# open-flash/swf-renderer

Measured on AMD Instinct MI355X. Metric: Mpixels/sec rasterized @ 4K, 10k-edge synthetic shape set, higher is better.
Workload: dtype i32+f64(exact integers)/u8

## Files before the change

### swf_renderer_amd/csrc/device_types.hpp

```cpp
#pragma once

#include <stdint.h>

#include "../../include/swfr.h"

namespace swfr {

constexpr int TILE_W = 64;
constexpr int TILE_H = 16;
constexpr int STRIP_H = 8;
constexpr int STRIPS_PER_TILE = TILE_H / STRIP_H;

struct DevEdge {
    int32_t ytop, ybot;
    int32_t x1, y1;
    int32_t dir;
    int32_t pad;
    int64_t ex;
    int64_t dy;
    int64_t dq, dr;
    double inv_dy;
    double inv_dx;
    int64_t fr;
    int64_t r15;
    int32_t fq, q15;
};
static_assert(sizeof(DevEdge) == 96, "DevEdge layout");

struct FastEdge {
    int32_t x1, a0, DX, D;
    double invD;
    int32_t q15, r15;
    int32_t hq, hr;
    int32_t dqf, drf;
    int32_t ytop, ybot;
    int32_t dir, fq;
    double invW, fr;
};
static_assert(sizeof(FastEdge) == 80, "FastEdge layout");

using DevPath = swfr_path;

enum : uint32_t { ROW_EMPTY = 0, ROW_FULL = 1, ROW_SUB = 2 };
constexpr uint32_t REC_FULL = 0x80000000u;
constexpr uint32_t REC_CELLS = 0x40000000u;
constexpr int ROWS_CHUNK = 64;

enum : uint32_t { PATH_OP_MASK = 0x0fu, PATH_OP_LERP = 0x10u, PATH_OP_GROUP_BEGIN = 0x20u, PATH_OP_GROUP_END = 0x40u, PATH_OP_MASKED = 0x80u };
enum : uint32_t { BE_BOXES = 1u, BE_LERP = 2u, BE_SOLID = 4u, BE_OPAQUE_COVER = 8u  };

struct ChunkInfo {
    uint32_t path, first_row, rec_base, rows;
    uint32_t slot0;
    uint32_t first_edge, n_edges;
    uint32_t pad;
};

struct BandSlot {
    uint32_t path;
    uint32_t slot;
    uint32_t band;
    uint32_t pad;
};

struct DevBitmap {
    const uint32_t* pixels;
    uint32_t width, height;
};

struct DevFilter {
    int32_t on, cw, ch, xbits, ybits;
    uint32_t x_off, y_off;
    int32_t m00, m01, m10, m11;
    int32_t pad;
    int64_t base_x, base_y;
    const uint32_t* pixels;
    uint32_t width, height;
    uint32_t extend;
    uint32_t kind;
    uint32_t nearest;
    uint32_t pad2;
};
static_assert(sizeof(DevFilter) == 96, "DevFilter layout");

struct DevGradient {
    int64_t base_x, base_y;
    int32_t m00, m01, m10, m11;
    int32_t c1x, c1y, c1r, dx, dy, dr;
    int32_t n_intervals, extend;
    double a, inva, mindr;
    int32_t x[SWFR_MAX_STOPS + 2];
    float ramp[SWFR_MAX_STOPS + 1][8];
    uint16_t col[SWFR_MAX_STOPS + 2][4];
    int32_t x_min, pad;
};

struct Cell {
    uint32_t w;
};
static_assert(sizeof(Cell) == 4, "Cell layout");
constexpr int MAX_PATH_WIDTH = 8192;
constexpr int CELL_H = 16384;
constexpr Cell make_cell_v(int col_rel, int v) { return Cell{((uint32_t)col_rel << 19) | ((uint32_t)v & 0x7ffffu)}; }
constexpr Cell make_cell(int col_rel, int ch, int ua) { return make_cell_v(col_rel, ch * CELL_H + ua); }
constexpr int cell_col(Cell c) { return (int)(c.w >> 19); }
constexpr int cell_ua(Cell c) { return (int)(c.w << 18) >> 18; }
constexpr int cell_ch(Cell c) { return (((int)(c.w << 13) >> 13) - cell_ua(c)) >> 14; }
constexpr int MAX_CELLS_PER_EDGE_ROW = 17;

struct RowInfo2 {
    uint32_t off;
    uint16_t n;
    uint16_t mode;
};
enum : uint32_t { ROW_DEFER = 3,
                  ROW_FOREIGN = 4 };

struct BandEntry2 {
    int16_t x_min, x_max, y_min, y_max;
    uint32_t flags;
    uint32_t solid;
    uint32_t style;
    uint32_t first_edge, n_edges;
    uint32_t path;
};
static_assert(sizeof(BandEntry2) == 32, "BandEntry2 layout");

struct SlowRow {
    uint32_t path;
    int32_t row;
    uint32_t ri;
    uint32_t pad;
};

enum : uint32_t { C2_ERROR = 0, C2_SLOW = 1, C2_HUGE = 2, C2_TIE_ROWS = 3, C2_TIE_PAIRTEST_SKIPPED = 4, C2_TIE_SORT_OVERFLOW = 5, C2_TIE_DEPTH = 6,
                  C2_CELLS = 7, C2_HEAD = 8 , C2_PATHQ = 16,
                  C2_SLOWQ = 16 , C2_HUGEQ = 20 , C2_WORDS = 32 };
constexpr uint32_t SLOW_PASSES = 4;
constexpr uint32_t C2_HEADS = 8;
// ... 57 lines not shown
```

### swf_renderer_amd/csrc/frame_layout.hpp

```cpp
#pragma once
#include <stddef.h>
#include <stdint.h>

#include "device_types.hpp"

namespace swfr {

inline size_t pad256(size_t bytes) { return (bytes + 255) & ~size_t(255); }

struct FrameDims {
    size_t n_edges = 0, n_paths = 0, n_slots = 0, n_rows = 0, n_chunks = 0, n_strips = 0, n_strip_slots = 0, cell_total = 0;
    template <class Layout>
    static FrameDims of_layout(const Layout& L, size_t n_edges, size_t n_paths) {
        return FrameDims{n_edges, n_paths, L.n_slots, L.n_rows, L.n_chunks, L.n_strips, L.n_strip_slots, L.cell_total};
    }

    size_t edge_count() const { return 2 * n_edges + 1; }
    size_t band_entry_count() const { return n_slots; }
    size_t row_count() const { return n_slots * TILE_H + 64; }
    size_t cell_count() const { return cell_total; }
    size_t slow_count() const { return 2 * (n_rows + 64); }
    size_t path_word_count() const { return n_paths + 64; }
    size_t chunk_count() const { return n_chunks + 1; }
    size_t band_slot_count() const { return n_slots + 8; }
    size_t strip_count() const { return n_strip_slots + 1; }
    size_t strip_cost_count() const { return n_strips + 1; }
};

template <class V>
void for_each_frame_buffer_parity(Frame2& f, const FrameDims& d, V&& v) {
    v(f.edges, d.edge_count(), true); v(f.band_list, d.band_entry_count(), true); v(f.rows, d.row_count(), false); v(f.cells, d.cell_count(), false);
    v(f.slow, d.slow_count(), false); v(f.huge, d.slow_count(), false); v(f.path_flag, d.path_word_count(), true); v(f.path_queue, d.path_word_count(), false);
    v(f.chunks, d.chunk_count(), true); v(f.band_slots, d.band_slot_count(), true); v(f.strips, d.strip_count(), true); v(f.strip_cost, d.strip_cost_count(), true);
    v(f.counters, size_t(C2_WORDS), true);
}
template <class V>
void for_each_frame_buffer(Frame2& f, const FrameDims& d, V&& v) {
    for_each_frame_buffer_parity(f, d, [&](auto*& p, size_t n, bool) { v(p, n); });
}
inline uint8_t* carve_frame(Frame2& f, const FrameDims& d, uint8_t* base) {
    for_each_frame_buffer(f, d, [&](auto*& p, size_t n) { p = reinterpret_cast<decltype(p + 0)>(base); base += pad256(n * sizeof(*p)); });
    return base;
}
inline size_t frame_work_bytes(const FrameDims& d) {
    Frame2 f{};
    size_t bytes = 0;
    for_each_frame_buffer(f, d, [&](auto* p, size_t n) { bytes += pad256(n * sizeof(*p)); });
    return bytes;
}

inline uint8_t* carve_frame_ahead(Frame2& f, const FrameDims& d, uint8_t* base) {
    for_each_frame_buffer_parity(f, d, [&](auto*& p, size_t n, bool per_parity) {
        if (per_parity) { p = reinterpret_cast<decltype(p + 0)>(base); base += pad256(n * sizeof(*p)); }
    });
    return base;
}
inline size_t frame_ahead_bytes(const FrameDims& d) {
    Frame2 f{};
    size_t bytes = 0;
    for_each_frame_buffer_parity(f, d, [&](auto* p, size_t n, bool per_parity) { if (per_parity) bytes += pad256(n * sizeof(*p)); });
    return bytes;
}

inline size_t cls_bytes_of(size_t n_slots, size_t tiles_x) { return (size_t(STRIPS_PER_TILE) * n_slots * tiles_x + 64 + 15) & ~size_t(15); }
inline size_t cls_region_bytes(size_t n_slots, size_t tiles_x, size_t n_strips) { return cls_bytes_of(n_slots, tiles_x) + (n_strips + 1) * sizeof(StripTop); }
inline size_t cls_region_bytes(const FrameDims& d, size_t tiles_x) { return cls_region_bytes(d.n_slots, tiles_x, d.n_strips); }
inline void set_cls_region(Frame2& f, const FrameDims& d, size_t tiles_x, uint8_t* base) {
    f.cls = base;
    f.strip_top = reinterpret_cast<StripTop*>(base + cls_bytes_of(d.n_slots, tiles_x));
}

}
```

### swf_renderer_amd/csrc/raster2.hip

```cpp
#include "raster_common.hip"

namespace swfr {

__device__ __forceinline__ void lds_barrier() {
#ifdef SWFR_EMU
    __syncthreads();
#else
    __builtin_amdgcn_fence(__ATOMIC_RELEASE, "workgroup", "local");
    __builtin_amdgcn_s_barrier();
    __builtin_amdgcn_fence(__ATOMIC_ACQUIRE, "workgroup", "local");
#endif
}

#ifdef SWFR_EMU
typedef const Frame2* FramePtr;
#define FRAME_PTR(frames, i) ((frames) + (i))
#else
typedef const Frame2 __attribute__((address_space(4)))* FramePtr;
#define FRAME_PTR(frames, i) ((FramePtr)((frames) + (i)))
#endif

#ifdef SWFR_TSTATS
#define TRACE_WGS 32768
__device__ uint32_t swfr_trace_buf[3][TRACE_WGS][8];
// ... 56 lines not shown
    if (ix2 < ix1) { int t = ix1; ix1 = ix2; ix2 = t; t = f1; f1 = f2; f2 = t; int32_t tq = q1; q1 = q2; q2 = tq; int64_t tr = r1; r1 = r2; r2 = tr; }
    const int span = ix2 - ix1 + 1;
    const int64_t dx = (int64_t)(q2 - q1) * edy + (r2 - r1);
    const int64_t t0 = ((int64_t)((ix1 + 1) * 256 - q1) * edy - r1) * 15;
    int64_t yq, yr;
    floor_div_inv(t0, dx, inv_dx, yq, yr);
    const int64_t fq = fq0, fr = fr0;
#ifdef SWFR_EMU
    {
        int64_t cq, cr2; floor_div(15ll * 256 * edy, dx, cq, cr2);
        int64_t dq2, dr2; floor_div(t0, dx, dq2, dr2);
        if (cq != fq || cr2 != fr || dq2 != yq || dr2 != yr || inv_dx != 1.0 / (double)dx) { std::fprintf(stderr, "full_cells: per-edge row constants disagree\n"); std::abort(); }
    }
#endif
    int y_prev = (int)yq;
    if (span <= MAX_CELLS_PER_EDGE_ROW) {
        put_cell_h(dst, ix1, sign * y_prev, 256 + f1, xminp, xmaxp);
#pragma unroll 1
        for (int k = 1; k < span - 1; ++k) {
            yq += fq; yr += fr; if (yr >= dx) { ++yq; yr -= dx; }
            const int h = (int)yq - y_prev;
            put_cell_h(dst + k, ix1 + k, sign * h, 256, xminp, xmaxp);
            y_prev = (int)yq;
        }
        put_cell_h(dst + span - 1, ix2, sign * (15 - y_prev), f2, xminp, xmaxp);
        return;
    }
    int n = 0;
    if (y_prev) put_cell_h(dst + n++, ix1, sign * y_prev, 256 + f1, xminp, xmaxp);
#pragma unroll 1
    for (int c = ix1 + 1; c < ix2; ++c) {
        yq += fq; yr += fr; if (yr >= dx) { ++yq; yr -= dx; }
        const int h = (int)yq - y_prev;
        if (h && n < MAX_CELLS_PER_EDGE_ROW - 1) put_cell_h(dst + n++, c, sign * h, 256, xminp, xmaxp);
        y_prev = (int)yq;
    }
    if (15 - y_prev) put_cell_h(dst + n++, ix2, sign * (15 - y_prev), f2, xminp, xmaxp);
    while (n < MAX_CELLS_PER_EDGE_ROW) put_cell(dst + n++, xminp, 0, 0, xminp, xmaxp);
}
__device__ __forceinline__ void sub_cell(Cell* __restrict__ dst, int x, int sgn, int xminp, int xmaxp) {
    put_cell(dst, x >> 8, sgn, sgn * 2 * (x & 255), xminp, xmaxp);
}
__device__ __forceinline__ uint32_t alloc_cells(FramePtr FR, uint32_t n, int lane) {
    uint32_t base = 0;
    if (lane == 0 && n) {
        const uint32_t old = atomicAdd(&FR->counters[C2_HEAD], n);
        base = FR->cell_main + old;
        if ((uint64_t)base + n > FR->cell_slice) { atomicOr(&FR->counters[C2_ERROR], E2_CELL_ARENA); base = ~0u; }
    }
    return (uint32_t)__builtin_amdgcn_readfirstlane((int)base);
}

__device__ __forceinline__ const swfr_style& style_at(FramePtr FR, uint32_t i) {
    return *reinterpret_cast<const swfr_style*>(reinterpret_cast<const char*>(FR->styles) + (size_t)i * FR->style_stride);
}
__device__ __forceinline__ BandEntry2 make_band_entry2(const DevPath& P, uint32_t p, uint32_t band, FramePtr FR) {
    BandEntry2 e;
    e.x_min = (int16_t)P.x_min; e.x_max = (int16_t)P.x_max; e.y_min = (int16_t)P.y_min; e.y_max = (int16_t)P.y_max;
    e.style = P.style; e.first_edge = P.first_edge; e.n_edges = P.n_edges; e.path = p;
    const uint32_t kind = style_at(FR, P.style).kind, pixel = style_at(FR, P.style).pixel;
    uint32_t fl = 0;
    if (P.kind == SWFR_PATH_BOXES) fl |= BE_BOXES;
    if (P.lerp) fl |= BE_LERP;
    if (kind == SWFR_STYLE_SOLID) fl |= BE_SOLID;
    if (kind == SWFR_STYLE_SOLID && P.lerp && (pixel >> 24) == 0xffu) fl |= BE_OPAQUE_COVER;
    e.flags = fl | (band << 8); e.solid = pixel;
    return e;
}
__device__ __forceinline__ bool path_has_area(const DevPath& P) { return P.y_max > P.y_min && P.x_max > P.x_min; }
__device__ __forceinline__ uint32_t path_chunk_count(const DevPath& P, uint32_t chunk_rows, uint32_t& a0) {
    a0 = (uint32_t)P.y_min / TILE_H * TILE_H;
    if (P.kind != SWFR_PATH_TOR || P.y_max <= P.y_min) return 0u;
    return ((uint32_t)P.y_max - a0 + chunk_rows - 1) / chunk_rows;
}

template <uint32_t BIN_THREADS> __device__ __forceinline__ void order_body(FramePtr F, uint32_t xcd_class);
constexpr uint32_t BAND_PER_THREAD = 16;
#ifndef BIN_ORDER_FIRST_SMALL
#define BIN_ORDER_FIRST_SMALL 1
#endif
#ifndef BIN_ORDER_FIRST_LARGE
#define BIN_ORDER_FIRST_LARGE 0
#endif
template <uint32_t BIN_THREADS, bool ORDER_FIRST> __device__ __forceinline__ void bin_body(FramePtr F, uint32_t slow_kernels) {
    constexpr uint32_t BAND_LIST = 4 * BIN_THREADS;
    static_assert(BIN_THREADS % 64 == 0 && BIN_THREADS >= (uint32_t)C2_WORDS, "whole wavefronts; block 0 clears the counters in one step");
    __shared__ uint32_t wave_cnt[BIN_THREADS / 64];
    __shared__ uint32_t band_hits[BAND_LIST];
    const int tid = threadIdx.x, lane = tid & 63, wave = tid >> 6;
    if (blockIdx.x == 0 && tid < C2_WORDS) F->counters[tid] = 0;
    const uint32_t order_at = ORDER_FIRST ? 0u : gridDim.x - XCDS;
    if (blockIdx.x - order_at < XCDS) { order_body<BIN_THREADS>(F, blockIdx.x - order_at); return; }
    const uint32_t block = blockIdx.x - (ORDER_FIRST ? XCDS : 0u);
    if (block < F->n_bands) {
        const int band = (int)block;
        const uint32_t b0 = F->band_off[band], n_b = F->band_off[band + 1] - b0;
        uint32_t n = 0;
        const uint32_t n_paths = F->n_paths;
        for (uint32_t base = 0; base < n_paths && n < n_b; base += BAND_PER_THREAD * BIN_THREADS) {
            const uint32_t p0 = base + (uint32_t)tid * BAND_PER_THREAD;
            uint32_t mask = 0;
            if (p0 < n_paths) {
                const uint4* t4 = reinterpret_cast<const uint4*>(F->path_bands + p0);
                const uint4 q[4] = {t4[0], t4[1], t4[2], t4[3]};
#pragma unroll
                for (int k = 0; k < 4; ++k) {
                    const uint32_t v[4] = {q[k].x, q[k].y, q[k].z, q[k].w};
#pragma unroll
                    for (int i = 0; i < 4; ++i) if ((v[i] & 0xffffu) <= (uint32_t)band && (uint32_t)band <= (v[i] >> 16)) mask |= 1u << (4 * k + i);
                }
            }
            const uint32_t cnt = (uint32_t)__popc(mask);
            const uint32_t incl = (uint32_t)wave_scan_incl((int)cnt);
            if (lane == 63) wave_cnt[wave] = incl;
            __syncthreads();
            uint32_t before = 0, total = 0;
            for (int w = 0; w < (int)(BIN_THREADS / 64); ++w) { const uint32_t t = wave_cnt[w]; if (w < wave) before += t; total += t; }
            const uint32_t first = before + incl - cnt;
            for (uint32_t lo = 0; lo < total; lo += BAND_LIST) {
                uint32_t m = mask, idx = first;
                while (m) {
                    const uint32_t bit = (uint32_t)__ffs((int)m) - 1u; m &= m - 1u;
                    if (idx >= lo && idx < lo + BAND_LIST) band_hits[idx - lo] = p0 + bit;
                    ++idx;
                }
                __syncthreads();
                const uint32_t in_window = min(total - lo, BAND_LIST);
                uint32_t local_trow = 0;
                const bool own = owns_band(F, band, local_trow);
                const int ty0 = band * TILE_H, tile_y1 = min(ty0 + TILE_H, F->height);
                for (uint32_t ib = 0; ib < in_window; ib += BIN_THREADS) {
                    const uint32_t i = ib + (uint32_t)tid;
                    uint32_t p = 0, at = 0;
                    bool valid = i < in_window;
                    if (valid) { p = band_hits[i]; at = n + lo + i; valid = at < n_b; }
                    int x_min = 0, x_max = 0;
                    uint32_t e_flags = 0, e_solid = 0, p_first = 0, p_nedges = 0;
                    bool box = false;
                    if (valid) {
                        const DevPath P = F->paths[p];
                        const uint32_t slot = b0 + at;
                        const BandEntry2 e = make_band_entry2(P, p, (uint32_t)band, F);
                        F->band_list[slot] = e;
                        BandSlot bs; bs.path = p; bs.slot = slot; bs.band = (uint32_t)band; bs.pad = 0;
                        F->band_slots[F->path_slots[p] + (uint32_t)(band - P.y_min / TILE_H)] = bs;
                        box = P.kind == SWFR_PATH_BOXES;
                        x_min = P.x_min; x_max = P.x_max; e_flags = e.flags; e_solid = e.solid; p_first = P.first_edge; p_nedges = P.n_edges;
                    }
                    for (unsigned long long bm = __ballot(box); bm; bm &= bm - 1ull) {
                        const int src = __ffsll((long long)bm) - 1;
                        const uint32_t b_at = (uint32_t)__shfl((int)at, src), b_flags = (uint32_t)__shfl((int)e_flags, src), b_solid = (uint32_t)__shfl((int)e_solid, src);
                        const uint32_t b_first = (uint32_t)__shfl((int)p_first, src), b_nedges = (uint32_t)__shfl((int)p_nedges, src);
                        const int b_xmin = __shfl(x_min, src), b_xmax = __shfl(x_max, src);
                        uint8_t* out = F->cls + (size_t)STRIPS_PER_TILE * F->tiles_x * b0 + b_at;
                        const uint32_t opq = (b_flags & BE_OPAQUE_COVER) ? CLS_OPAQUE : 0u;
                        const swfr_edge bx = F->raw[b_first];
                        const bool one_box = b_nedges == 1 && bx.y1 <= ty0 * 256 && bx.y2 >= tile_y1 * 256;
                        const int tc_a = b_xmin / TILE_W, tc_b = (b_xmax - 1) / TILE_W;
                        const int items = (tc_b - tc_a + 1) * STRIPS_PER_TILE;
                        for (int k = lane; k < items; k += 64) {
                            const int tc = tc_a + k / STRIPS_PER_TILE, sp = k % STRIPS_PER_TILE;
                            const int tx0 = tc * TILE_W, tile_x1 = min(tx0 + TILE_W, F->width);
                            uint32_t f = CLS_BOX | CLS_NONEMPTY | CLS_NOTFULL;
                            if (one_box && bx.x1 <= tx0 * 256 && bx.x2 >= tile_x1 * 256) f = CLS_NONEMPTY | opq;
                            out[(size_t)(tc * STRIPS_PER_TILE + sp) * n_b] = (uint8_t)f;
                            if (own && ty0 + sp * STRIP_H < F->height) strip_top_note(F, (local_trow * (uint32_t)F->tiles_x + (uint32_t)tc) * STRIPS_PER_TILE + (uint32_t)sp, b_at + 1u, f, b_solid);
                        }
                    }
                }
                __syncthreads();
            }
            n += total;
            __syncthreads();
        }
        if (n != n_b && tid == 0) atomicOr(&F->counters[C2_ERROR], E2_ROW_TABLE);
        return;
    }
    const uint32_t rel = block - F->n_bands, edge_blocks = F->mono ? 0u : (F->n_edges + BIN_THREADS - 1) / BIN_THREADS;
    const bool path_block = rel >= edge_blocks;
    const uint32_t i = path_block ? ~0u : rel * BIN_THREADS + (uint32_t)tid;
    if (i < F->n_edges) {
        const swfr_edge e = F->raw[i];
        const DevPath EP = F->paths[e.reserved];
        if (slow_kernels) F->edges[i] = make_dev_edge(e, EP);
        const FastEdge fe = make_fast_edge(e, EP);
        fast_edges_of(F->edges, F->n_edges)[i] = fe;
#ifdef SWFR_EMU
        const DevEdge de = make_dev_edge(e, EP);
        if (de.ytop != fe.ytop || de.ybot != fe.ybot) { std::fprintf(stderr, "FastEdge span disagrees with DevEdge\n"); std::abort(); }
        if (de.ybot > de.ytop && de.dy) {
            const int probe[3] = {de.ytop, (de.ytop + de.ybot) / 2, de.ybot};
            for (int t = 0; t < 3; ++t) {
                int32_t q0, q1, r1; int64_t r0;
                edge_x_at(de, probe[t], q0, r0);
                fast_x_at(fe.a0, fe.DX, fe.D, fe.invD, probe[t], q1, r1);
                if (q0 != fe.x1 + q1 || r0 != 256ll * r1) { std::fprintf(stderr, "fast_x_at disagrees with edge_x_at\n"); std::abort(); }
            }
            int64_t tq = fe.dqf, tr = fe.drf;
            if (fe.DX < 0 && tr != 0) { tq += 1; tr -= fe.D; }
            if (tq != de.dq || 256 * tr != de.dr || (e.y2 - e.y1 >= 200 && (fe.q15 != de.q15 || 256ll * fe.r15 != de.r15)) || fe.fq != de.fq) { std::fprintf(stderr, "FastEdge constants disagree with DevEdge\n"); std::abort(); }
        }
#endif
    }
    const uint32_t ip = path_block ? (rel - edge_blocks) * BIN_THREADS + (uint32_t)tid : ~0u;
    if (!path_block) return;
    uint32_t nc = 0, a0 = 0, c0 = 0, inc0 = 0, slots0 = ~0u, first_edge = 0, n_path_edges = 0, band0 = 0;
    if (ip < F->n_paths) {
        const DevPath P = F->paths[ip];
        F->path_flag[ip] = 0;
        nc = path_chunk_count(P, F->chunk_rows, a0);
        c0 = F->path_chunks[ip]; inc0 = F->path_inc[ip];
        slots0 = path_has_area(P) ? F->path_slots[ip] : ~0u;
        first_edge = P.first_edge; n_path_edges = P.n_edges; band0 = (uint32_t)P.y_min / TILE_H;
    }
    auto write_chunk = [&](uint32_t path, uint32_t c, uint32_t a0_, uint32_t c0_, uint32_t inc0_, uint32_t slots0_, uint32_t fe_, uint32_t ne_, uint32_t band0_) {
        ChunkInfo ck;
        ck.path = path; ck.first_row = a0_ + c * F->chunk_rows; ck.rec_base = inc0_; ck.rows = F->chunk_rows;
        ck.slot0 = slots0_ != ~0u ? slots0_ + (ck.first_row / TILE_H - band0_) : ~0u;
        ck.first_edge = fe_; ck.n_edges = ne_; ck.pad = 0;
        if (c0_ + c < F->chunk_cap) F->chunks[c0_ + c] = ck;
    };
    constexpr uint32_t OWN_CHUNKS = 8;
    if (nc <= OWN_CHUNKS)
        for (uint32_t c = 0; c < nc; ++c) write_chunk(ip, c, a0, c0, inc0, slots0, first_edge, n_path_edges, band0);
    for (unsigned long long big = __ballot(nc > OWN_CHUNKS); big; big &= big - 1ull) {
        const int src = __ffsll((long long)big) - 1;
        const uint32_t b_nc = (uint32_t)__shfl((int)nc, src), b_path = (uint32_t)__shfl((int)ip, src), b_a0 = (uint32_t)__shfl((int)a0, src);
        const uint32_t b_c0 = (uint32_t)__shfl((int)c0, src), b_inc0 = (uint32_t)__shfl((int)inc0, src), b_slots0 = (uint32_t)__shfl((int)slots0, src);
        const uint32_t b_fe = (uint32_t)__shfl((int)first_edge, src), b_ne = (uint32_t)__shfl((int)n_path_edges, src), b_band0 = (uint32_t)__shfl((int)band0, src);
        for (uint32_t c = (uint32_t)lane; c < b_nc; c += 64u) write_chunk(b_path, c, b_a0, b_c0, b_inc0, b_slots0, b_fe, b_ne, b_band0);
    }
}
constexpr uint32_t ORDER_RANGES = 8;
__device__ __forceinline__ uint32_t order_range(uint32_t cost) {
    return cost >= 48u ? 0u : cost >= 32u ? 1u : cost >= 24u ? 2u : cost >= 16u ? 3u : cost >= 8u ? 4u : cost >= 4u ? 5u : cost >= 1u ? 6u : 7u;
}
constexpr uint32_t ORDER_U = 16;
template <uint32_t BIN_THREADS> __device__ __forceinline__ void order_body(FramePtr F, uint32_t x) {
    constexpr uint32_t ROWINFO = BIN_THREADS >= BIN_THREADS_SMALL ? 256u : 32u;
    __shared__ uint2 rowinfo[ROWINFO];
    __shared__ uint32_t cnt[ORDER_RANGES][ORDER_U][BIN_THREADS / 64];
    const int tid = threadIdx.x, lane = tid & 63, wave = tid >> 6;
    const uint32_t n_strips = F->n_strips, bc = F->band_stride, bi = F->band_first;
    const uint32_t per_row = STRIPS_PER_TILE * (uint32_t)F->tiles_x;
    const uint32_t n_local = n_strips / per_row;
    const uint32_t rows_x = (n_local + XCDS - 1 - x) / XCDS, max_rows = (n_local + XCDS - 1) / XCDS;
    const uint32_t n_mine = rows_x * per_row;
    const bool by_cost = F->strip_order != 0u;
    for (uint32_t j = (uint32_t)tid; j < rows_x && j < ROWINFO; j += BIN_THREADS) {
        const uint32_t trow = (x + j * XCDS) * bc + bi, b0 = F->band_off[trow];
        rowinfo[j] = make_uint2(b0, F->band_off[trow + 1] - b0);
    }
    if (rows_x < max_rows)
        for (uint32_t j = (uint32_t)tid; j < per_row; j += BIN_THREADS) {
            StripDesc sd; sd.wg = ~0u; sd.band_begin = 0; sd.n_b = 0; sd.pad = 0;
            F->strips[(size_t)(n_mine + j) * XCDS + x] = sd;
        }
    __syncthreads();
    const uint32_t dq = BIN_THREADS / per_row, dr = BIN_THREADS - dq * per_row;
    auto advance = [&](uint32_t& j, uint32_t& pos) { j += dq; pos += dr; if (pos >= per_row) { pos -= per_row; ++j; } };
    auto strip_at = [&](uint32_t j, uint32_t pos) { return (x + j * XCDS) * per_row + pos; };
    for (uint32_t base = 0; base < n_mine; base += ORDER_U * BIN_THREADS) {
        const uint32_t n_round = min(n_mine - base, ORDER_U * BIN_THREADS), U = (n_round + BIN_THREADS - 1) / BIN_THREADS;
        unsigned long long ranges = 0;
        uint32_t behind[ORDER_U];
        const uint32_t i0 = base + (uint32_t)tid, j0 = i0 / per_row, pos0 = i0 - j0 * per_row;
        if (by_cost) {
            uint32_t c[ORDER_U];
            uint32_t j = j0, pos = pos0;
#pragma unroll
            for (uint32_t u = 0; u < ORDER_U; ++u) {
                c[u] = 0;
                if (u >= U) continue;
                const uint32_t i = base + u * BIN_THREADS + (uint32_t)tid;
                if (i < n_mine) c[u] = F->strip_cost[strip_at(j, pos)];
                advance(j, pos);
            }
            j = j0; pos = pos0;
#pragma unroll
            for (uint32_t u = 0; u < ORDER_U; ++u) {
                behind[u] = 0;
                if (u >= U) continue;
                const uint32_t i = base + u * BIN_THREADS + (uint32_t)tid;
                const bool valid = i < n_mine;
                if (valid && c[u]) F->strip_cost[strip_at(j, pos)] = 0;
                advance(j, pos);
                const uint32_t k = order_range(c[u]);
                ranges |= (unsigned long long)k << (3 * u);
                const uint32_t sh = 8u * (k & 3u), one = valid ? 1u << sh : 0u;
                const uint32_t lo = (uint32_t)wave_scan_incl((int)(k < 4u ? one : 0u)), hi = (uint32_t)wave_scan_incl((int)(k < 4u ? 0u : one));
                behind[u] = (((k < 4u ? lo : hi) >> sh) & 0xffu) - 1u;
                const uint32_t tot_lo = (uint32_t)__builtin_amdgcn_readlane((int)lo, 63), tot_hi = (uint32_t)__builtin_amdgcn_readlane((int)hi, 63);
                if (lane < (int)ORDER_RANGES) cnt[lane][u][wave] = ((lane < 4 ? tot_lo : tot_hi) >> (8 * (lane & 3))) & 0xffu;
            }
            __syncthreads();
            if (tid < 64) {
                uint32_t* flat = &cnt[0][0][0];
                uint32_t carry = 0;
                for (uint32_t q = 0; q < ORDER_RANGES; ++q)
                    for (uint32_t e0 = 0; e0 < U * (BIN_THREADS / 64); e0 += 64) {
                        const uint32_t e = e0 + (uint32_t)tid, lim = U * (BIN_THREADS / 64);
                        const uint32_t v = e < lim ? flat[q * ORDER_U * (BIN_THREADS / 64) + e] : 0u;
                        const uint32_t incl = (uint32_t)wave_scan_incl((int)v);
                        if (e < lim) flat[q * ORDER_U * (BIN_THREADS / 64) + e] = carry + incl - v;
                        carry += (uint32_t)__builtin_amdgcn_readlane((int)incl, 63);
                    }
            }
            __syncthreads();
        } else {
#pragma unroll
            for (uint32_t u = 0; u < ORDER_U; ++u) behind[u] = 0;
        }
        uint32_t j = j0, pos = pos0;
#pragma unroll
        for (uint32_t u = 0; u < ORDER_U; ++u) {
            if (u >= U) continue;
            const uint32_t i = base + u * BIN_THREADS + (uint32_t)tid;
            if (i < n_mine) {
                uint32_t rank = i;
                if (by_cost) rank = base + cnt[(uint32_t)(ranges >> (3 * u)) & 7u][u][wave] + behind[u];
                uint2 ri;
                if (j < ROWINFO) ri = rowinfo[j]; else { const uint32_t trow = (x + j * XCDS) * bc + bi, b0 = F->band_off[trow]; ri = make_uint2(b0, F->band_off[trow + 1] - b0); }
                StripDesc sd; sd.wg = strip_at(j, pos); sd.band_begin = ri.x; sd.n_b = ri.y; sd.pad = (pos / STRIPS_PER_TILE) | ((x + j * XCDS) << 16);
                F->strips[(size_t)rank * XCDS + x] = sd;
            }
            advance(j, pos);
        }
        __syncthreads();
    }
}
__global__ __launch_bounds__(1024) __attribute__((amdgpu_num_sgpr(80))) void k2_bin_b(const Frame2* __restrict__ frames, uint32_t slow_kernels) { TRACE_DECL; TRACE_NOWAIT(0); bin_body<BIN_THREADS_LARGE, BIN_ORDER_FIRST_LARGE != 0>(FRAME_PTR(frames, blockIdx.y), slow_kernels); TRACE(7); TRACE_OUT(0, blockIdx.x); }
__global__ __launch_bounds__(256) void k2_bin_small_b(const Frame2* __restrict__ frames, uint32_t slow_kernels) { TRACE_DECL; TRACE_NOWAIT(0); bin_body<BIN_THREADS_SMALL, BIN_ORDER_FIRST_SMALL != 0>(FRAME_PTR(frames, blockIdx.y), slow_kernels); TRACE(7); TRACE_OUT(0, blockIdx.x); }

__device__ __forceinline__ uint32_t pack_sub_cell(int x, int sgn, int xminp, int xmaxp) {
    int col = x >> 8, f = x & 255, live = 1;
    if (col >= xmaxp) { col = xmaxp - 1; f = 0; live = 0; }
    else if (col < xminp) { col = xminp; f = 0; }
    const int v = live * CELL_H + 2 * f, neg = sgn < 0 ? -1 : 0;
    return make_cell_v(col - xminp, (v ^ neg) - neg).w;
}

#include "rows3.hip"

#ifndef R2_WAVES
#define R2_WAVES 5
#endif
#define R2_ATTR __attribute__((amdgpu_waves_per_eu(R2_WAVES)))
#ifndef R2_WIDE_WAVES
#define R2_WIDE_WAVES 3
#endif
__global__ __launch_bounds__(64) R2_ATTR void k2_rows_b(const Frame2* __restrict__ frames) {
    FramePtr FR = FRAME_PTR(frames, blockIdx.y);
    if (blockIdx.x >= FR->n_chunks) return;
    rows3_chunk_body<ROWS_STAGE, ROWS_FAST_N>(FR, blockIdx.x);
}
__global__ __launch_bounds__(64) __attribute__((amdgpu_waves_per_eu(R2_WIDE_WAVES))) void k2_rows_wide_b(const Frame2* __restrict__ frames) {
    FramePtr FR = FRAME_PTR(frames, blockIdx.y);
    if (blockIdx.x >= FR->n_chunks) return;
    rows3_chunk_body<ROWS_STAGE_WIDE, ROWS_FAST_WIDE>(FR, blockIdx.x);
}
__global__ __launch_bounds__(64) R2_ATTR void k2_rows_ahead_b(const Frame2* __restrict__ frames, const Frame2* __restrict__ ahead, uint32_t n_ahead, uint32_t ahead_frames) {
    if (blockIdx.x < n_ahead) {
        if (blockIdx.y >= ahead_frames) return;
        TRACE_DECL; TRACE_NOWAIT(0);
        bin_body<BIN_THREADS_AHEAD, true>(FRAME_PTR(ahead, blockIdx.y), 0u);
        TRACE(7); TRACE_OUT(0, blockIdx.x);
        return;
    }
    FramePtr FR = FRAME_PTR(frames, blockIdx.y);
    const uint32_t chunk = blockIdx.x - n_ahead;
    if (chunk >= FR->n_chunks) return;
    rows3_chunk_body<ROWS_STAGE, ROWS_FAST_N>(FR, chunk);
}

#include "mono.hip"

__global__ __launch_bounds__(64) void k2_rows_mono_b(const Frame2* __restrict__ frames) {
    FramePtr FR = FRAME_PTR(frames, blockIdx.y);
    if (blockIdx.x >= FR->n_chunks) return;
    mono_chunk_body(FR, blockIdx.x);
}
__global__ __launch_bounds__(HUGE_THREADS) void k2_rows_mono_huge_b(const Frame2* __restrict__ frames) { mono_huge_loop(FRAME_PTR(frames, blockIdx.y)); }


__device__ __forceinline__ void sort_pairs(uint16_t* __restrict__ dst, const int* __restrict__ cell, int p, int cnt) {
    const int x = 2 * p, y = 2 * p + 1;
    if (y < cnt) { const bool keep = cell[x] <= cell[y]; dst[x] = (uint16_t)(keep ? x : y); dst[y] = (uint16_t)(keep ? y : x); }
    else if (x < cnt) dst[x] = (uint16_t)x;
}
__device__ __forceinline__ void merge_step(const uint16_t* __restrict__ src, uint16_t* __restrict__ dst, const int* __restrict__ cell, int s, int width, int cnt) {
    const int a1 = min(s + width, cnt), b1 = min(s + 2 * width, cnt);
    int ia = s, ib = a1, o = s;
    if (ib >= b1) { while (ia < a1) dst[o++] = src[ia++]; return; }
    bool phase_a = cell[src[ia]] <= cell[src[ib]];
    for (;;) {
        if (phase_a) {
            const int x = cell[src[ib]];
            while (ia < a1 && cell[src[ia]] <= x) dst[o++] = src[ia++];
            if (ia == a1) { while (ib < b1) dst[o++] = src[ib++]; return; }
        }
        const int x = cell[src[ia]];
        while (ib < b1 && cell[src[ib]] <= x) dst[o++] = src[ib++];
        if (ib == b1) { while (ia < a1) dst[o++] = src[ia++]; return; }
        phase_a = true;
    }
}

#define START_MAX 8192
__device__ __forceinline__ void rank_tmp(DevEdge* E, int i, int rank) { E[i].pad = rank; }
#define START_LDS 1024
__device__ __forceinline__ void start_ranks_body(FramePtr FR, uint32_t p) {
    __shared__ int sort_cell[START_MAX];
    __shared__ uint16_t sort_a[START_MAX], sort_b[START_MAX];
    __shared__ uint32_t member[START_MAX];
    __shared__ int yt_l[START_LDS], mark_l[START_LDS];
    __shared__ uint32_t wave_cnt[4];
    __shared__ int next_y;
    const int tid = threadIdx.x, lane = tid & 63, wave = tid >> 6;
    const DevPath P = FR->paths[p];
    if (P.kind != SWFR_PATH_TOR) return;
    DevEdge* E = FR->edges + P.first_edge;
    const int ne = (int)P.n_edges;
    const bool staged = ne <= START_LDS;
    auto start_row = [&](int i) { if (staged) return yt_l[i]; const int yt = E[i].ytop; return E[i].ybot > yt ? yt : INT_MAX; };
    auto mark = [&](int i) { return staged ? mark_l[i] : E[i].pad; };
    if (staged) {
        for (int i = tid; i < ne; i += 256) { const int yt = E[i].ytop; yt_l[i] = E[i].ybot > yt ? yt : INT_MAX; }
        __syncthreads();
    }
    for (int i = tid; i < ne; i += 256) {
        const int yt = start_row(i);
        int cnt = 0, partner = -1;
        if (yt != INT_MAX)
            for (int j = 0; j < ne; ++j)
                if (j != i && start_row(j) == yt) { ++cnt; partner = j; }
        int rank = 0;
        if (cnt == 1) {
            const DevEdge a = E[i], b = E[partner];
            int ca = a.x1, cb = b.x1;
            if (a.dy) { int32_t q; int64_t rm; edge_x_at(a, yt, q, rm); ca = cell_of(q, rm, a.dy); }
            if (b.dy) { int32_t q; int64_t rm; edge_x_at(b, yt, q, rm); cb = cell_of(q, rm, b.dy); }
            rank = i < partner ? (ca <= cb ? 0 : 1) : (cb <= ca ? 1 : 0);
        } else if (cnt > 1) rank = -1;
        rank_tmp(E, i, rank);
        if (staged) mark_l[i] = rank;
    }
    __syncthreads();
    int done_y = INT_MIN;
    for (;;) {
        if (tid == 0) next_y = INT_MAX;
        __syncthreads();
        for (int i = tid; i < ne; i += 256) {
            const int yt = start_row(i);
            if (yt != INT_MAX && mark(i) == -1 && yt > done_y) atomicMin(&next_y, yt);
        }
// ... 1185 lines not shown
                            for (int j = 0; j < 8; ++j) px[j] = solid;
                            continue;
                        }
                        const uint32_t cv0 = g >= row_lo && g < row_hi ? 255u : 0u, cv1 = g + 4 >= row_lo && g + 4 < row_hi ? 255u : 0u;
#pragma unroll
                        for (int j = 0; j < 4; ++j) { al[j] = cv0; al[4 + j] = cv1; }
                    }
#ifdef ABL_T_NOBLEND
                    for (int j = 0; j < 8; ++j) px[j] = al[j] == 255u ? solid : px[j];
#else
                    if constexpr (SHADERS >= 3) {
                        if (op) { blend8_op<SHADERS == 7>(px, al, op, eflags, solid, styles, style, bitmaps, cx0, cy0); continue; }
                    }
                    blend8<SHADERS>(px, al, eflags, solid, styles, style, bitmaps, cx0, cy0, bq, lane);
#endif
                }
                lds_barrier();
            }
        }
        TRACE_NOWAIT(6);
#pragma unroll
        for (int j = 0; j < 8; ++j) {
            const uint32_t p = px[j];
#ifdef SWFR_EMU
            px[j] = (p & 0xff00ff00u) | ((p >> 16) & 0xffu) | ((p & 0xffu) << 16);
#else
            px[j] = __builtin_amdgcn_perm(p, p, 0x03000102u);
#endif
        }
        uint32_t* const fbp = fb_to ? fb_to : FR->fb;
        const bool vec_ok = (width & 3) == 0 && ((uintptr_t)fbp & 15u) == 0u;
        if (vec_ok && tx0 + TILE_W <= width && ty0 + STRIP_H <= height) {
            typedef uint32_t row4 __attribute__((vector_size(16)));
            uint32_t* rowp = fbp + (size_t)cy0 * (size_t)width + cx0;
            *reinterpret_cast<row4*>(rowp) = row4{px[0], px[1], px[2], px[3]};
            *reinterpret_cast<row4*>(rowp + 4 * (size_t)width) = row4{px[4], px[5], px[6], px[7]};
        } else {
#pragma unroll
            for (int h = 0; h < 2; ++h) {
                const int y = cy0 + 4 * h;
                if (y >= height) continue;
                uint32_t* rowp = fbp + (size_t)y * (size_t)width + cx0;
                if (vec_ok && cx0 + 4 <= width) *reinterpret_cast<uint4*>(rowp) = make_uint4(px[4 * h], px[4 * h + 1], px[4 * h + 2], px[4 * h + 3]);
                else {
#pragma unroll
                    for (int i = 0; i < 4; ++i) if (cx0 + i < width) rowp[i] = px[4 * h + i];
                }
            }
        }
        TRACE(7);
        TRACE_OUT(2, w);
    }
}


#ifndef T2_WAVES
#define T2_WAVES 7
#endif
__global__ __launch_bounds__(64) __attribute__((amdgpu_waves_per_eu(T2_WAVES))) void k2_tiles_solid_b(const Frame2* __restrict__ frames, uint32_t* fb_to) { tiles3_body<0>(FRAME_PTR(frames, blockIdx.y), fb_to); }
#ifndef T2_WAVES_SHADED
#define T2_WAVES_SHADED 4
#endif
__global__ __launch_bounds__(64) __attribute__((amdgpu_waves_per_eu(T2_WAVES_SHADED))) void k2_tiles_bitmap_b(const Frame2* __restrict__ frames, uint32_t* fb_to) { tiles3_body<1>(FRAME_PTR(frames, blockIdx.y), fb_to); }
__global__ __launch_bounds__(64) __attribute__((amdgpu_waves_per_eu(T2_WAVES_SHADED))) void k2_tiles_shaded_b(const Frame2* __restrict__ frames, uint32_t* fb_to) { tiles3_body<2>(FRAME_PTR(frames, blockIdx.y), fb_to); }
__global__ __launch_bounds__(64) __attribute__((amdgpu_waves_per_eu(T2_WAVES_BLEND))) void k2_tiles_blend_b(const Frame2* __restrict__ frames, uint32_t* fb_to) { tiles3_body<3>(FRAME_PTR(frames, blockIdx.y), fb_to); }
__global__ __launch_bounds__(64) __attribute__((amdgpu_waves_per_eu(T2_WAVES_LAYER))) void k2_tiles_layer_b(const Frame2* __restrict__ frames, uint32_t* fb_to) { tiles3_body<4>(FRAME_PTR(frames, blockIdx.y), fb_to); }
__global__ __launch_bounds__(64) __attribute__((amdgpu_waves_per_eu(T2_WAVES_LAYER))) void k2_tiles_mask_b(const Frame2* __restrict__ frames, uint32_t* fb_to) { tiles3_body<5>(FRAME_PTR(frames, blockIdx.y), fb_to); }
__global__ __launch_bounds__(64) __attribute__((amdgpu_waves_per_eu(T2_WAVES_LAYER))) void k2_tiles_fade_b(const Frame2* __restrict__ frames, uint32_t* fb_to) { tiles3_body<6>(FRAME_PTR(frames, blockIdx.y), fb_to); }
__global__ __launch_bounds__(64) __attribute__((amdgpu_waves_per_eu(T2_WAVES_LAYER))) void k2_tiles_alpha_b(const Frame2* __restrict__ frames, uint32_t* fb_to) { tiles3_body<7>(FRAME_PTR(frames, blockIdx.y), fb_to); }

void launch2_bin(hipStream_t st, const Frame2* frames, uint32_t n_frames, uint32_t max_edges, uint32_t max_paths, uint32_t max_bands, uint32_t slow_kernels, bool mono, uint32_t bin_threads) {
    const uint32_t T = bin_threads == BIN_THREADS_SMALL ? BIN_THREADS_SMALL : BIN_THREADS_LARGE;
    const uint32_t g = XCDS + max_bands + (mono ? 0u : (max_edges + T - 1) / T) + (max_paths + T - 1) / T;
    if (T == BIN_THREADS_SMALL) hipLaunchKernelGGL(k2_bin_small_b, dim3(g, n_frames), dim3(BIN_THREADS_SMALL), 0, st, frames, slow_kernels);
    else hipLaunchKernelGGL(k2_bin_b, dim3(g, n_frames), dim3(BIN_THREADS_LARGE), 0, st, frames, slow_kernels);
}
bool rows_wide_instance(uint32_t max_path_edges, bool wide) { return wide || max_path_edges > ROWS_STAGE; }
void launch2_rows(hipStream_t st, const Frame2* frames, uint32_t n_frames, uint32_t max_chunks, uint32_t max_path_edges, bool wide, bool mono) {
    if (!max_chunks) return;
    if (mono) { hipLaunchKernelGGL(k2_rows_mono_b, dim3(max_chunks, n_frames), dim3(64), 0, st, frames); return; }
    if (rows_wide_instance(max_path_edges, wide)) hipLaunchKernelGGL(k2_rows_wide_b, dim3(max_chunks, n_frames), dim3(64), 0, st, frames);
    else hipLaunchKernelGGL(k2_rows_b, dim3(max_chunks, n_frames), dim3(64), 0, st, frames);
}
void launch2_rows_ahead(hipStream_t st, const Frame2* frames, const Frame2* ahead, uint32_t n_frames, uint32_t ahead_frames, uint32_t max_edges, uint32_t max_paths, uint32_t max_bands, uint32_t max_chunks) {
    constexpr uint32_t T = BIN_THREADS_AHEAD;
    const uint32_t n_ahead = XCDS + max_bands + (max_edges + T - 1) / T + (max_paths + T - 1) / T;
    hipLaunchKernelGGL(k2_rows_ahead_b, dim3(n_ahead + max_chunks, n_frames), dim3(64), 0, st, frames, ahead, n_ahead, ahead_frames);
}
void launch2_rows_slow(hipStream_t st, const Frame2* frames, uint32_t n_frames, uint32_t grid_slow, uint32_t grid_huge, uint32_t max_passes, bool mono) {
    if (mono) { hipLaunchKernelGGL(k2_rows_mono_huge_b, dim3(grid_huge ? grid_huge : 64u, n_frames), dim3(HUGE_THREADS), 0, st, frames); return; }
    if (grid_slow) hipLaunchKernelGGL(k2_start_ranks_b, dim3(grid_slow / 4 + 1, n_frames), dim3(256), 0, st, frames);
    for (uint32_t pass = 0; pass < SLOW_PASSES; ++pass) {
        if (grid_slow) hipLaunchKernelGGL(k2_rows_slow_b, dim3(grid_slow, n_frames), dim3(64), 0, st, frames, pass);
        if (grid_huge) hipLaunchKernelGGL(k2_rows_huge_b, dim3(grid_huge, n_frames), dim3(HUGE_THREADS), 0, st, frames, pass);
        if (pass + 1 >= max_passes) break;
    }
}
__device__ __forceinline__ void linear_pieces_body(FramePtr FR) {
    if (blockIdx.x >= FR->n_linear_records) return;
    const DevGradient* G = FR->src.gradients + blockIdx.x;
    if (G->pad <= 0) return;
    int32_t* table = const_cast<int32_t*>(FR->src.fparams) + (G->pad - 1);
    const uint32_t path = (uint32_t)table[-1];
    if (path >= FR->n_paths) return;
    const DevPath P = FR->paths[path];
    const int per_row = G->dr, run = 256;
    const int xmax = P.x_max - P.x_min;
    for (int r = P.y_min + (int)threadIdx.x; r < P.y_max; r += (int)blockDim.x) {
        int32_t* out = table + (size_t)(r - G->c1r) * (size_t)per_row;
        int n_out = 0;
        const BandSlot bs = FR->band_slots[FR->path_slots[path] + (uint32_t)(r / TILE_H - P.y_min / TILE_H)];
        RowInfo2 ri; ri.off = 0; ri.n = 0; ri.mode = (uint16_t)ROW_FOREIGN;
        if (bs.path == path && bs.band == (uint32_t)(r / TILE_H)) ri = FR->rows[(size_t)bs.slot * TILE_H + (uint32_t)(r & (TILE_H - 1))];
        int n = (int)ri.n;
        if (bs.path != path || bs.band != (uint32_t)(r / TILE_H)) n = 0;
        if (ri.mode == ROW_FOREIGN || ri.mode == ROW_DEFER) n = 0;
        if (ri.off > FR->cell_slice - min((uint32_t)n, FR->cell_slice)) n = 0;
        const Cell* cp = FR->cells + ri.off;
        bool have = false, first = true;
        int sx = 0, scov = 0, x0 = 0, x1 = 0;
        auto piece = [&](int from) { if (n_out < per_row) out[n_out] = from + P.x_min; ++n_out; };
        auto feed = [&](int x, int raw) {
            if (have) {
                const int len = x - sx, cov = (int)(((uint32_t)(17 * scov + 256) >> 9) & 255u);
                if (first) { x0 = x1 = sx; first = false; }
                if (len > 1) {
                    if (len >= run && cov == 255) { if (x1 != x0) piece(x0); piece(sx); x0 = x; }
                    else if (cov == 0 && x1 - x0 > run) { piece(x0); x0 = x; }
                }
                x1 = x;
            }
            have = true; sx = x; scov = raw;
        };
        int prev_x = 0, last_x = -1, cover = 0, last_cover = 0, cur = -1;
        for (;;) {
            int c = 0x7fffffff;
            for (int k = 0; k < n; ++k) { const int col = cell_col(cp[k]); if (col > cur && col < c) c = col; }
            if (c >= xmax) break;
            int hsum = 0, usum = 0;
            for (int k = 0; k < n; ++k) if (cell_col(cp[k]) == c) { hsum += cell_ch(cp[k]); usum += cell_ua(cp[k]); }
            if (c > prev_x && cover != last_cover) { feed(prev_x, cover); last_cover = cover; last_x = prev_x; }
            cover += hsum * 512;
            const int area = cover - usum;
            if (area != last_cover) { feed(c, area); last_cover = area; last_x = c; }
            prev_x = c + 1;
            cur = c;
        }
        if (prev_x <= xmax && cover != last_cover) { feed(prev_x, cover); last_cover = cover; last_x = prev_x; }
        if (last_x < xmax && last_cover) feed(xmax, 0);
        if (!first && x1 != x0) piece(x0);
        if (n_out > per_row) { atomicOr(&FR->counters[C2_ERROR], E2_ROW_TABLE); n_out = per_row; }
        for (int k = n_out; k < per_row; ++k) out[k] = 0x7fffffff;
    }
}
__global__ __launch_bounds__(64) void k2_linear_pieces_b(const Frame2* __restrict__ frames) { linear_pieces_body(FRAME_PTR(frames, blockIdx.y)); }
void launch2_linear_pieces(hipStream_t st, const Frame2* frames, uint32_t n_frames, uint32_t n_gradients) {
    if (!n_gradients) return;
    hipLaunchKernelGGL(k2_linear_pieces_b, dim3(n_gradients, n_frames), dim3(64), 0, st, frames);
}
void launch2_tiles(hipStream_t st, const Frame2* frames, uint32_t n_frames, uint32_t max_strips, uint32_t grid_cap, int shader_level, uint32_t* fb_to) {
    if (!max_strips) return;
    uint32_t g = max_strips < grid_cap ? max_strips : grid_cap;
    if (grid_cap == ~0u && max_strips > T3_PAIR_FROM) g = (max_strips + 1u) / 2u;
    if (shader_level >= 7) hipLaunchKernelGGL(k2_tiles_alpha_b, dim3(g, n_frames), dim3(64), 0, st, frames, fb_to);
    else if (shader_level == 6) hipLaunchKernelGGL(k2_tiles_fade_b, dim3(g, n_frames), dim3(64), 0, st, frames, fb_to);
    else if (shader_level == 5) hipLaunchKernelGGL(k2_tiles_mask_b, dim3(g, n_frames), dim3(64), 0, st, frames, fb_to);
    else if (shader_level == 4) hipLaunchKernelGGL(k2_tiles_layer_b, dim3(g, n_frames), dim3(64), 0, st, frames, fb_to);
    else if (shader_level == 3) hipLaunchKernelGGL(k2_tiles_blend_b, dim3(g, n_frames), dim3(64), 0, st, frames, fb_to);
    else if (shader_level >= 2) hipLaunchKernelGGL(k2_tiles_shaded_b, dim3(g, n_frames), dim3(64), 0, st, frames, fb_to);
    else if (shader_level == 1) hipLaunchKernelGGL(k2_tiles_bitmap_b, dim3(g, n_frames), dim3(64), 0, st, frames, fb_to);
// ... 17 lines not shown
```

### swf_renderer_amd/csrc/raster_common.hip

```cpp
#include <hip/hip_runtime.h>
#include <stdint.h>
#include <type_traits>
#ifdef SWFR_EMU
#include <cstdio>
#include <cstdlib>
#endif

#include "device_types.hpp"

#ifdef SWFR_EMU
#define SWFR_OPAQUE(x) asm volatile("" : "+r"(x))
#else
#define SWFR_OPAQUE(x) asm volatile("" : "+v"(x))
#endif
#ifdef SWFR_EMU
#define SWFR_PIN_SGPR(x) do { } while (0)
#define SWFR_GLOBAL_PTR(T) T*
#else
#define SWFR_PIN_SGPR(x) asm volatile("" : "+s"(x))
#define SWFR_GLOBAL_PTR(T) T __attribute__((address_space(1)))*
#endif

namespace swfr {

__device__ __forceinline__ void floor_div(int64_t a, int64_t b, int64_t& q, int64_t& r) {
    q = (int64_t)floor((double)a / (double)b);
    r = a - q * b;
    while (r < 0) { --q; r += b; }
    while (r >= b) { ++q; r -= b; }
}
__device__ __forceinline__ void floor_div_inv(int64_t a, int64_t b, double inv_b, int64_t& q, int64_t& r) {
    q = (int64_t)(int32_t)floor((double)a * inv_b);
    r = a - q * b;
    while (r < 0) { --q; r += b; }
    while (r >= b) { ++q; r -= b; }
}
__device__ __forceinline__ void trunc_div(int64_t a, int64_t b, int64_t& q, int64_t& r) {
    floor_div(a, b, q, r);
    if (a < 0 && r != 0) { ++q; r -= b; }
}
__device__ __forceinline__ void edge_x_at(const DevEdge& e, int s, int32_t& quo, int64_t& rem) {
    if (e.dy == 0) { quo = e.x1; rem = 0; return; }
    const int64_t a = ((int64_t)(2 * s + 1) << 8) - 30 * (int64_t)e.y1;
    int64_t q, r;
    floor_div_inv(a * e.ex, e.dy, e.inv_dy, q, r);
    quo = e.x1 + (int32_t)q;
    rem = r;
}
__device__ __forceinline__ int cell_of(int32_t quo, int64_t rem, int64_t dy) { return quo + (rem >= dy / 2 ? 1 : 0); }
__device__ __forceinline__ uint32_t clamp_col(int c) { return (uint32_t)min(max(c, 0), 65535); }
__device__ __forceinline__ int record_height(uint32_t roles) {
    if (roles & REC_CELLS) return (int)(int8_t)(roles >> 8);
    if (roles & REC_FULL) return (roles & 1u) ? 15 : -15;
    return __popc(roles & 0x15555555u) - __popc(roles & 0x2aaaaaaau);
}

__device__ __forceinline__ int mul_i24(int a, int b) {
#ifdef SWFR_EMU
    return a * b;
#else
    int r;
    asm("v_mul_i32_i24 %0, %1, %2" : "=v"(r) : "v"(a), "v"(b));
    return r;
#endif
}
template <int SH>
__device__ __forceinline__ int lshl_add(int a, int b) {
#ifdef SWFR_EMU
    return (int)(((uint32_t)a << SH) + (uint32_t)b);
#else
    int r;
    asm("v_lshl_add_u32 %0, %1, %2, %3" : "=v"(r) : "v"(a), "i"(SH), "v"(b));
    return r;
#endif
}
#ifdef SWFR_EMU
__device__ __forceinline__ uint32_t pk_mad_u16(uint32_t a, uint32_t b, uint32_t c) {
    return (((a & 0xffffu) * (b & 0xffffu) + (c & 0xffffu)) & 0xffffu) | ((((a >> 16) * (b >> 16) + (c >> 16)) & 0xffffu) << 16);
}
__device__ __forceinline__ uint32_t pk_add_u16(uint32_t a, uint32_t b) {
    return (((a & 0xffffu) + (b & 0xffffu)) & 0xffffu) | ((((a >> 16) + (b >> 16)) & 0xffffu) << 16);
}
template <int SH>
__device__ __forceinline__ uint32_t pk_lshr_u16(uint32_t a) { return ((a & 0xffffu) >> SH) | (((a >> 16) >> SH) << 16); }
#else
typedef unsigned short pk_u16x2 __attribute__((ext_vector_type(2)));
__device__ __forceinline__ uint32_t pk_mad_u16(uint32_t a, uint32_t b, uint32_t c) {
    return __builtin_bit_cast(uint32_t, (pk_u16x2)(__builtin_bit_cast(pk_u16x2, a) * __builtin_bit_cast(pk_u16x2, b) + __builtin_bit_cast(pk_u16x2, c)));
}
__device__ __forceinline__ uint32_t pk_add_u16(uint32_t a, uint32_t b) {
    return __builtin_bit_cast(uint32_t, (pk_u16x2)(__builtin_bit_cast(pk_u16x2, a) + __builtin_bit_cast(pk_u16x2, b)));
}
template <int SH>
__device__ __forceinline__ uint32_t pk_lshr_u16(uint32_t a) {
    return __builtin_bit_cast(uint32_t, (pk_u16x2)(__builtin_bit_cast(pk_u16x2, a) >> (unsigned short)SH));
}
#endif
__device__ __forceinline__ uint32_t pk_both(uint32_t f) { return f | (f << 16); }
__device__ __forceinline__ int wave_scan_incl(int v) {
    v += __builtin_amdgcn_update_dpp(0, v, 0x111, 0xf, 0xf, false);
    v += __builtin_amdgcn_update_dpp(0, v, 0x112, 0xf, 0xf, false);
    v += __builtin_amdgcn_update_dpp(0, v, 0x114, 0xf, 0xf, false);
    v += __builtin_amdgcn_update_dpp(0, v, 0x118, 0xf, 0xf, false);
    v += __builtin_amdgcn_update_dpp(0, v, 0x142, 0xa, 0xf, false);
    v += __builtin_amdgcn_update_dpp(0, v, 0x143, 0xc, 0xf, false);
    return v;
}

__device__ __forceinline__ DevEdge make_dev_edge(const swfr_edge& e, const DevPath& p) {
    DevEdge d;
    d.x1 = e.x1; d.y1 = e.y1; d.dir = e.dir; d.pad = 0; d.inv_dy = 0.0;
    d.inv_dx = 0.0; d.fr = 0; d.r15 = 0; d.fq = 0; d.q15 = 0;
    if (p.kind != SWFR_PATH_TOR) {
        d.ytop = d.ybot = 0; d.dy = 0; d.ex = 0; d.dq = d.dr = 0;
        return d;
    }
    int ytop = (int)((15ll * e.top + 128) >> 8), ybot = (int)((15ll * e.bottom + 128) >> 8);
    ytop = max(ytop, p.y_min * 15);
    ybot = min(ybot, p.y_max * 15);
    if (ybot <= ytop) { ytop = ybot = 0; }
    d.ytop = ytop; d.ybot = ybot;
    if (e.x1 == e.x2) {
        d.dy = 0; d.ex = 0; d.dq = d.dr = 0;
    } else {
        d.ex = (int64_t)(e.x2 - e.x1) * 256;
        d.dy = (int64_t)(e.y2 - e.y1) * 15 * 512;
        d.inv_dy = 1.0 / (double)d.dy;
        trunc_div(d.ex * 512, d.dy, d.dq, d.dr);
        const int64_t adx = (d.ex < 0 ? -d.ex : d.ex) * 7680;
        d.inv_dx = 1.0 / (double)adx;
        int64_t fq; floor_div_inv(3840 * d.dy, adx, d.inv_dx, fq, d.fr);
        d.fq = (int32_t)fq;
        if (e.y2 - e.y1 >= 200) {
            int64_t q15; floor_div_inv(d.ex * 7680, d.dy, d.inv_dy, q15, d.r15);
            d.q15 = (int32_t)q15;
        }
    }
    return d;
}

__device__ __forceinline__ FastEdge make_fast_edge(const swfr_edge& e, const DevPath& p) {
    FastEdge f;
    f.x1 = e.x1; f.a0 = 256 - 30 * e.y1; f.DX = 0; f.D = 30; f.invD = 1.0 / 30.0; f.q15 = f.r15 = f.hq = f.hr = f.dqf = f.drf = 0;
    {
        int ytop = (int)((15ll * e.top + 128) >> 8), ybot = (int)((15ll * e.bottom + 128) >> 8);
        ytop = max(ytop, p.y_min * 15);
        ybot = min(ybot, p.y_max * 15);
        if (ybot <= ytop) { ytop = ybot = 0; }
        f.ytop = ytop; f.ybot = ybot;
    }
    f.dir = e.dir; f.fq = 0; f.invW = 0.0; f.fr = 0.0;
    if (p.kind != SWFR_PATH_TOR || e.y2 <= e.y1) { f.ytop = f.ybot = 0; return f; }
    const int64_t DX = (int64_t)e.x2 - e.x1, D = 30ll * ((int64_t)e.y2 - e.y1);
    f.D = (int32_t)D; f.invD = 1.0 / (double)D;
    if (DX == 0) return f;
    f.DX = (int32_t)DX;
    int64_t q, r;
    floor_div_inv(512 * DX, D, f.invD, q, r);
    f.dqf = (int32_t)q; f.drf = (int32_t)r;
    int64_t tq = q, tr = r;
    if (DX < 0 && r != 0) { tq = q + 1; tr = r - D; }
    int64_t hq = tq / 2, hr = tr / 2;
    if (hr < 0) { --hq; hr += D; }
    f.hq = (int32_t)hq; f.hr = (int32_t)hr;
    if (e.y2 - e.y1 >= 200) {
        floor_div_inv(7680 * DX, D, f.invD, q, r);
        f.q15 = (int32_t)q; f.r15 = (int32_t)r;
    }
    const int64_t W = 512 * (DX < 0 ? -DX : DX);
    f.invW = 1.0 / (double)W;
    floor_div_inv(256 * D, W, f.invW, q, r);
    f.fq = (int32_t)q; f.fr = (double)r;
    return f;
}
__device__ __forceinline__ void fast_x_at(int32_t a0, int32_t DX, int32_t D, double invD, int s, int32_t& quo, int32_t& rem) {
    const double n = (double)(512 * s + a0) * (double)DX;
    const double qf = floor(n * invD);
    const double rf = fma(-qf, (double)D, n);
    int32_t q = (int32_t)qf, r = (int32_t)rf;
    if (r < 0) { --q; r += D; }
    if (r >= D) { ++q; r -= D; }
    quo = q; rem = r;
}
__device__ __forceinline__ FastEdge* fast_edges_of(DevEdge* edges, uint32_t n_edges) { return reinterpret_cast<FastEdge*>(edges + n_edges); }

#define CLS_PARTIAL 1u
#define CLS_NOTFULL 2u
#define CLS_NONEMPTY 4u
#define CLS_HOLE 16u
#define CLS_BOX 8u

#define ROWS_FAST_N 8
#define ROWS_FAST_WIDE 16
#define ROWS_BIG_MAXA 64
#ifndef ROWS_STAGE
#define ROWS_STAGE 32
#endif
#define ROWS_STAGE_WIDE 64

struct PathEdges {
    const DevEdge* dev; const swfr_edge* raw; const DevPath* P; bool from_raw;
    uint32_t* diag;
    __device__ __forceinline__ void limit_hit(uint32_t which) const { if (diag) atomicOr(&diag[which], 1u); }
    const RowInfo2* rows2; const BandSlot* band_slots; uint32_t bs0;
    uint32_t* retry;
    __device__ __forceinline__ uint32_t known_mode(int rho) const {
        if (!rows2 || rho < P->y_min || rho >= P->y_max) return ROW_DEFER;
        const BandSlot bs = band_slots[bs0 + (uint32_t)(rho / TILE_H - P->y_min / TILE_H)];
        return rows2[(size_t)bs.slot * TILE_H + (uint32_t)(rho & (TILE_H - 1))].mode;
    }
    __device__ __forceinline__ DevEdge operator()(uint32_t k) const { return from_raw ? make_dev_edge(raw[P->first_edge + k], *P) : dev[P->first_edge + k]; }
    __device__ __forceinline__ uint32_t size() const { return P->n_edges; }
    __device__ __forceinline__ void span(uint32_t k, int& ytop, int& ybot) const {
        if (!from_raw) { ytop = dev[P->first_edge + k].ytop; ybot = dev[P->first_edge + k].ybot; return; }
        const swfr_edge& e = raw[P->first_edge + k];
        ytop = max((int)((15ll * e.top + 128) >> 8), P->y_min * 15);
        ybot = min((int)((15ll * e.bottom + 128) >> 8), P->y_max * 15);
        if (ybot <= ytop) ytop = ybot = 0;
    }
};
__device__ __forceinline__ bool same_line(const DevEdge& a, const DevEdge& b) {
    return a.x1 == b.x1 && a.y1 == b.y1 && a.ex == b.ex && a.dy == b.dy;
}
#define NEW_SORT_MAX 16
__device__ __forceinline__ int sel_cell(const int (&v)[NEW_SORT_MAX], int i) {
    int r = v[0];
#pragma unroll
    for (int t = 1; t < NEW_SORT_MAX; ++t) r = (i == t) ? v[t] : r;
    return r;
}
__device__ __forceinline__ uint64_t merge_runs(uint64_t A, int na, uint64_t B, int nb, const int (&cell)[NEW_SORT_MAX]) {
    if (nb == 0) return A;
    if (na == 0) return B;
// ... 489 lines not shown
```

### swf_renderer_amd/csrc/renderer.cpp

```cpp
#include <hip/hip_runtime.h>

#include <algorithm>
#include <chrono>
#include <cfloat>
#include <cmath>
#include <cstdio>
#include <cstdlib>
#include <cstring>
#include <exception>
#include <map>
#include <memory>
#include <stdexcept>
#include <string>
#include <unordered_map>
#include <vector>

#include "../../include/swfr.h"
#include "device_types.hpp"
#include "frame_layout.hpp"
#include "frame_builder.hpp"
#include "shape_decoder.hpp"
#include "bitmap_decode.hpp"

namespace swfr {
void launch2_bin(hipStream_t, const Frame2*, uint32_t, uint32_t, uint32_t, uint32_t, uint32_t, bool, uint32_t);
void launch2_rows(hipStream_t, const Frame2*, uint32_t, uint32_t, uint32_t, bool, bool);
bool rows_wide_instance(uint32_t, bool);
void launch2_rows_ahead(hipStream_t, const Frame2*, const Frame2*, uint32_t, uint32_t, uint32_t, uint32_t, uint32_t, uint32_t);
void launch2_rows_slow(hipStream_t, const Frame2*, uint32_t, uint32_t, uint32_t, uint32_t, bool);
void launch2_tiles(hipStream_t, const Frame2*, uint32_t, uint32_t, uint32_t, int, uint32_t*);
void launch2_linear_pieces(hipStream_t, const Frame2*, uint32_t, uint32_t);
void launch_unpremultiply(hipStream_t, const uint32_t*, uint32_t*, size_t);
void launch_pack_band(hipStream_t, const uint32_t*, uint32_t*, int, int, uint32_t, uint32_t, uint32_t);
void launch_cxform_texels(hipStream_t, const uint8_t*, uint32_t*, size_t, const uint32_t*);
void launch_blur_capture(hipStream_t, const uint32_t*, uint32_t*, size_t);
void launch_blur_pass(hipStream_t, const uint32_t*, uint32_t*, uint32_t, uint32_t, uint32_t, bool);
void launch_shadow_alpha(hipStream_t, const uint32_t*, uint32_t*, uint32_t, uint32_t, int32_t, int32_t);
void launch_shadow_finish(hipStream_t, const uint32_t*, const uint32_t*, bool, uint32_t*, size_t, uint32_t, uint32_t, uint32_t);
}

using namespace swfr;

namespace {

constexpr size_t COUNTER_WORDS = C2_WORDS;

struct HipError {
    hipError_t code;
    const char* what;
};
#define HIP_CHECK(expr)                                 \
    do {                                                \
        hipError_t _e = (expr);                         \
        if (_e != hipSuccess) throw HipError{_e, #expr}; \
    } while (0)

template <class T>
struct DevBuf {
    T* ptr = nullptr;
    size_t cap = 0;
    void reserve(size_t n) {
        if (n <= cap) return;
        if (ptr) HIP_CHECK(hipFree(ptr));
        ptr = nullptr;
        cap = 0;
        size_t want = std::max<size_t>(n, 64);
        want += want / 2;
        HIP_CHECK(hipMalloc(reinterpret_cast<void**>(&ptr), want * sizeof(T)));
        cap = want;
    }
    void release() {
        if (ptr) (void)hipFree(ptr);
        ptr = nullptr;
        cap = 0;
    }
};

struct SceneView { const swfr_edge* edges; size_t n_edges; const swfr_path* paths; size_t n_paths; const swfr_style* styles; size_t n_styles; };

struct LaunchPlan {
    uint32_t max_edges, max_paths, max_bands, slow_kernels;
    uint32_t bin_threads;
    uint32_t max_chunks, max_path_edges; bool rows_wide;
    bool run_slow; uint32_t grid_slow, grid_huge, slow_passes;
    uint32_t linear_grid;
    uint32_t max_strips, tiles_grid; int shader_level;
};

struct SceneArena {
    uint8_t* dev = nullptr;
    uint8_t* host = nullptr;
    size_t cap = 0, used = 0;
    hipEvent_t copied = nullptr;
    hipEvent_t copy_begin = nullptr, copy_end = nullptr;
    void begin(size_t bytes) {
        if (copied) HIP_CHECK(hipEventSynchronize(copied));
        if (bytes > cap) {
            if (dev) (void)hipFree(dev);
            if (host) (void)hipHostFree(host);
            dev = host = nullptr;
            const size_t want = bytes + bytes / 2 + 4096;
            HIP_CHECK(hipMalloc(reinterpret_cast<void**>(&dev), want));
            HIP_CHECK(hipHostMalloc(reinterpret_cast<void**>(&host), want, hipHostMallocDefault));
            cap = want;
        }
        used = 0;
    }
    static size_t padded(size_t bytes) { return (bytes + 255) & ~size_t(255); }
    void* push(const void* src, size_t bytes) {
        void* d = dev + used;
        if (bytes && src) std::memcpy(host + used, src, bytes);
        used += padded(bytes);
        return d;
    }
    void flush(hipStream_t st, bool timed = false) {
        if (timed) {
            if (!copy_begin) { HIP_CHECK(hipEventCreate(&copy_begin)); HIP_CHECK(hipEventCreate(&copy_end)); }
            HIP_CHECK(hipEventRecord(copy_begin, st));
        }
        if (used) HIP_CHECK(hipMemcpyAsync(dev, host, used, hipMemcpyHostToDevice, st));
        if (timed) HIP_CHECK(hipEventRecord(copy_end, st));
        if (!copied) HIP_CHECK(hipEventCreateWithFlags(&copied, hipEventDisableTiming));
        HIP_CHECK(hipEventRecord(copied, st));
    }
    void release() {
        if (copied) (void)hipEventDestroy(copied);
        if (copy_begin) { (void)hipEventDestroy(copy_begin); (void)hipEventDestroy(copy_end); }
        if (dev) (void)hipFree(dev);
        if (host) (void)hipHostFree(host);
        dev = host = nullptr; copied = nullptr; copy_begin = copy_end = nullptr; cap = used = 0;
    }
};

struct DeviceBitmap {
    uint32_t* pixels = nullptr;
    uint32_t width = 0, height = 0;
    uint64_t gen = 0;
    std::vector<uint8_t> straight;
    uint8_t* d_straight = nullptr;
    hipEvent_t straight_ready = nullptr;
    hipStream_t straight_stream = nullptr;
    bool straight_done = false;
    bool captured = false;
};

struct CxVariant {
    uint32_t* pixels = nullptr;
    size_t bytes = 0;
    uint32_t bitmap = 0;
    uint64_t gen = 0;
    hipEvent_t ready = nullptr;
    hipStream_t stream = nullptr;
    bool done = false;
    bool pinned = false;
    uint64_t used_epoch = 0, last_use = 0;
    std::shared_ptr<uint32_t> table;
};

}

struct swfr_renderer {
    uint32_t width = 0, height = 0;
    swfr_config cfg{};
    bool has_device = false;
    std::string error;
    std::unique_ptr<FrameBuilder> builder;
    std::string json_scratch;

    hipStream_t stream = nullptr;
    uint32_t* h_counters = nullptr;
    std::vector<hipEvent_t> ev;
    struct Scene {
        SceneArena arena;
        FrameDims dims;
        LaunchPlan bounds{};
        Frame2 proto{};
        Frame2* frames_dev = nullptr;
        Frame2* frames_ahead = nullptr;
        uint32_t slow_passes = SLOW_PASSES;
        bool slow_verified = false;
        int slow_state = 0;
    };
    Scene scn[4];
    struct FrameSet {
        hipStream_t stream = nullptr;
        DevBuf<uint8_t> work, cls;
        DevBuf<uint32_t> strip_cost;
        DevBuf<uint32_t> strip_cost_ahead;
        uint32_t* counters = nullptr;
        DevBuf<uint32_t> d_fb;
        hipGraph_t graph = nullptr;
        hipGraphExec_t graph_exec = nullptr;
        uint64_t graph_key = 0;
    };
    FrameSet fs[4];
    uint64_t scene_gen = 0;
    int resident_batch = 2;
#ifdef SWFR_EMU
    int use_graphs = 0;
#else
    int use_graphs = 0;
#endif
    DevBuf<DevBitmap> d_bitmap_table;
    DevBuf<uint32_t> d_tmp;
    DevBuf<uint32_t> d_counters;
    int in_flight = 4;
    bool scene_from_builder = false;
    uint32_t sets_ready = 0;
    int hint_slow_state = 0; uint32_t hint_slow_passes = SLOW_PASSES;
    uint32_t* fb_cur = nullptr;
    std::map<uint32_t, DeviceBitmap> bitmaps;
    std::vector<DevBitmap> bitmap_table;
    uint64_t bitmap_gen = 0;
    std::unordered_map<std::string, CxVariant> cx_cache;
    size_t cx_bytes = 0, cx_budget = size_t(512) << 20;
    uint64_t cx_epoch = 0, cx_tick = 0, cx_synced_epoch = ~uint64_t(0);
    std::vector<std::string> cx_pins;
    std::vector<DevBitmap> variant_table;
    DevBuf<uint32_t> blur_tex[SWFR_MAX_BLUR_LAYERS];
    DevBuf<uint32_t> blur_scratch;
    DevBuf<uint32_t> shadow_scratch;
    std::vector<DevBitmap> blur_table;
    bool bitmap_table_dirty = false, bitmap_table_dirty_copied = false;
    bool scene_ready = false, fb_valid = false;
    swfr_timing timing{};
    swfr_path_timing path_timing{};
    int force_chunk_rows = 0;
    int strip_order = 1;
    int event_stride = 16;
    bool event_stride_given = false;
    bool mono = false;
    int fast_limit = 16;
    int tiles_grid = 0;
    int bin_threads = 0;
    uint32_t last_bin_threads = 0;
    int bin_ahead = 1;
    uint32_t last_ahead_launches = 0;
    int tiles_shaders = 0;
    bool rows_wide = false;
    struct BatchGroup {
        SceneArena arena;
        DevBuf<uint8_t> work, cls;
        hipStream_t stream = nullptr;
        uint32_t* h_counters = nullptr;
        size_t h_counters_cap = 0;
        hipEvent_t ev_begin = nullptr, ev_end = nullptr;
    };
    BatchGroup groups[2];
    int batch_frames = 64;
    uint32_t* targets[4] = {nullptr, nullptr, nullptr, nullptr};
    swfr_stats stats = {};
    DevBuf<uint8_t> rb_work, rb_cls;
    DevBuf<Frame2> rb_frames;
    DevBuf<uint32_t> rb_fb;
    hipEvent_t rb_ev[2] = {nullptr, nullptr};
    uint8_t* h_image = nullptr; size_t h_image_cap = 0;
    hipEvent_t read_done = nullptr;
    bool read_pending = false;
    uint32_t n_targets = 0, async_next = 0, async_used = 0;

    ~swfr_renderer() {
        if (has_device) {
            (void)hipSetDevice(cfg.device);
            d_bitmap_table.release(); d_tmp.release(); d_counters.release();
            rb_work.release(); rb_cls.release(); rb_frames.release(); rb_fb.release();
            for (auto& t : blur_tex) t.release();
            blur_scratch.release(); shadow_scratch.release();
            for (auto& e : rb_ev) if (e) (void)hipEventDestroy(e);
            if (h_image) (void)hipHostFree(h_image);
            if (read_done) (void)hipEventDestroy(read_done);
            for (int k = 0; k < 4; ++k) {
                FrameSet& x = fs[k];
                x.work.release(); x.cls.release(); x.strip_cost.release(); x.strip_cost_ahead.release(); x.d_fb.release();
                if (x.graph_exec) (void)hipGraphExecDestroy(x.graph_exec);
                if (x.graph) (void)hipGraphDestroy(x.graph);
                if (k > 0 && x.stream) (void)hipStreamDestroy(x.stream);
                scn[k].arena.release();
            }
            if (h_counters) (void)hipHostFree(h_counters);
            for (auto& g : groups) {
                g.arena.release(); g.work.release(); g.cls.release();
                if (g.stream) (void)hipStreamDestroy(g.stream);
                if (g.h_counters) (void)hipHostFree(g.h_counters);
                if (g.ev_begin) { (void)hipEventDestroy(g.ev_begin); (void)hipEventDestroy(g.ev_end); }
            }
            for (auto& kv : bitmaps) {
                if (kv.second.pixels) (void)hipFree(kv.second.pixels);
                if (kv.second.d_straight) (void)hipFree(kv.second.d_straight);
                if (kv.second.straight_ready) (void)hipEventDestroy(kv.second.straight_ready);
            }
            for (auto& kv : cx_cache) {
                if (kv.second.pixels) (void)hipFree(kv.second.pixels);
                if (kv.second.ready) (void)hipEventDestroy(kv.second.ready);
            }
            for (auto& e : ev) if (e) (void)hipEventDestroy(e);
            if (stream) (void)hipStreamDestroy(stream);
        }
    }
};

namespace {

int fail(swfr_renderer* r, int code, const std::string& msg) {
    if (r) r->error = msg;
    return code;
}

template <class F>
int guarded(swfr_renderer* r, F&& f) {
    try {
        if (r && r->has_device) HIP_CHECK(hipSetDevice(r->cfg.device));
        return f();
    } catch (const StatusError& e) {
        return fail(r, e.code, e.message);
    } catch (const HipError& e) {
        return fail(r, SWFR_ERR_DEVICE, std::string(e.what) + ": " + hipGetErrorString(e.code));
    } catch (const std::bad_alloc&) {
        return fail(r, SWFR_ERR_CAPACITY, "out of host memory");
    } catch (const std::exception& e) {
// ... 749 lines not shown
                r->cx_cache.erase(it);
                throw;
            }
        } else {
            CxVariant& e = it->second;
            if (!e.done && e.stream != st) {
                if (hipEventQuery(e.ready) == hipSuccess) e.done = true;
                else HIP_CHECK(hipStreamWaitEvent(st, e.ready, 0));
            }
        }
        CxVariant& e = it->second;
        e.used_epoch = r->cx_epoch;
        e.last_use = ++r->cx_tick;
        if (pin && !e.pinned) { e.pinned = true; r->cx_pins.push_back(key); }
        r->variant_table[k] = DevBitmap{e.pixels, bm.width, bm.height};
    }
}

struct FrameScratch { std::vector<swfr_edge> group_e, split_e; std::vector<swfr_path> group_p, split_p; std::vector<swfr_style> group_s; };
SceneView prepare_frame(swfr_renderer* r, SceneView a, hipStream_t st, bool pin, FrameScratch& S, SceneLayout& L) {
    bool faded = false;
    if (lower_groups(a, S.group_e, S.group_p, S.group_s, faded))
        a = SceneView{S.group_e.data(), S.group_e.size(), S.group_p.data(), S.group_p.size(), S.group_s.data(), S.group_s.size()};
    const SceneView drawn = a;
    const bool split = split_wide_paths(a, S.split_e, S.split_p);
    if (split) { a.edges = S.split_e.data(); a.n_edges = S.split_e.size(); a.paths = S.split_p.data(); a.n_paths = S.split_p.size(); }
    resolve_variants(r, drawn, st, pin);
    layout_scene(r, a, L, split ? &drawn : nullptr, faded);
    return a;
}

LaunchPlan plan_bounds(const SceneLayout& L, size_t n_edges, size_t n_paths) {
    LaunchPlan p{};
    p.max_edges = uint32_t(n_edges); p.max_paths = uint32_t(n_paths); p.max_bands = uint32_t(L.n_bands);
    p.max_chunks = uint32_t(L.n_chunks); p.max_path_edges = L.max_path_edges; p.rows_wide = L.rows_wide;
    p.linear_grid = L.n_linear ? uint32_t(L.gradients.size()) : 0u;
    p.max_strips = uint32_t(L.n_strip_slots); p.shader_level = L.shader_level;
    return p;
}
void merge_bounds(LaunchPlan& p, const LaunchPlan& q) {
    p.max_edges = std::max(p.max_edges, q.max_edges); p.max_paths = std::max(p.max_paths, q.max_paths); p.max_bands = std::max(p.max_bands, q.max_bands);
    p.max_chunks = std::max(p.max_chunks, q.max_chunks); p.max_path_edges = std::max(p.max_path_edges, q.max_path_edges); p.rows_wide = p.rows_wide || q.rows_wide;
    p.linear_grid = std::max(p.linear_grid, q.linear_grid); p.max_strips = std::max(p.max_strips, q.max_strips); p.shader_level = std::max(p.shader_level, q.shader_level);
}
void place_frame(Frame2& f, const FrameDims& d, size_t tiles_x, uint8_t*& w, uint8_t*& c) {
    w = carve_frame(f, d, w);
    set_cls_region(f, d, tiles_x, c);
    c += pad256(cls_region_bytes(d, tiles_x));
}
void place_frame_ahead(Frame2& f, const FrameDims& d, size_t tiles_x, uint8_t*& w, uint8_t*& c) {
    w = carve_frame_ahead(f, d, w);
    set_cls_region(f, d, tiles_x, c);
    c += pad256(cls_region_bytes(d, tiles_x));
}

int upload2(swfr_renderer* r, int si, bool all_sets, SceneView sv, uint32_t* fb_override, bool edges_tagged) {
    swfr_renderer::Scene& sc = r->scn[si];
    if (si == 0) r->scene_ready = false;
    if (r->async_used) {
        for (int k = 0; k < 4; ++k) if (r->fs[k].stream) HIP_CHECK(hipStreamSynchronize(r->fs[k].stream));
    }
    sc.slow_verified = false;
    sc.slow_state = si == 0 ? r->hint_slow_state : 0; sc.slow_passes = si == 0 ? r->hint_slow_passes : SLOW_PASSES;
    if (si > 0 && !r->fs[si].stream) HIP_CHECK(hipStreamCreateWithFlags(&r->fs[si].stream, hipStreamNonBlocking));
    const hipStream_t up_stream = r->fs[si].stream;
    const uint32_t tiles_x = (r->width + TILE_W - 1) / TILE_W;
    std::vector<swfr_edge> tagged;
    if (!edges_tagged) {
        tagged.assign(sv.edges, sv.edges + sv.n_edges);
        for (size_t i = 0; i < sv.n_paths; ++i)
            for (uint32_t k = 0; k < sv.paths[i].n_edges; ++k) tagged[sv.paths[i].first_edge + k].reserved = int32_t(i);
        if (r->mono)
            for (size_t i = 0; i < sv.n_paths; ++i)
                if (sv.paths[i].kind == SWFR_PATH_BOXES)
                    for (uint32_t k = 0; k < sv.paths[i].n_edges; ++k) round_box_to_pixels(tagged[sv.paths[i].first_edge + k]);
        sv.edges = tagged.data();
    }
    static thread_local FrameScratch scratch;
    static thread_local SceneLayout L;
    const SceneView a = prepare_frame(r, sv, up_stream, si == 0, scratch, L);
    const FrameDims dims = sc.dims = FrameDims::of_layout(L, a.n_edges, a.n_paths);
    sc.bounds = plan_bounds(L, a.n_edges, a.n_paths);
    SceneArena& A = sc.arena;
    A.begin(scene_arena_bytes(L, a) + SceneArena::padded(8 * sizeof(Frame2)) + 4096);
    Frame2 proto;
    std::memset(&proto, 0, sizeof proto);
    push_scene(A, L, a, proto);
    fill_frame_sizes(r, L, a, proto);
    if (r->bitmap_table_dirty) r->d_bitmap_table.reserve(r->bitmap_table.size());
    proto.src.bitmaps = r->d_bitmap_table.ptr;
    sc.proto = proto;
    const size_t cls_bytes = cls_region_bytes(dims, tiles_x);
    const int n_sets = std::max(1, std::min(r->in_flight, 4));
    const bool ahead = all_sets && r->bin_ahead && !r->mono && r->cfg.band_count <= 1;
    Frame2 fr[8];
    std::memset(fr, 0, sizeof fr);
    for (int k = 0; k < 4; ++k) {
        if (all_sets ? k >= n_sets : k != si) continue;
        auto& x = r->fs[k];
        Frame2& f = fr[k];
        f = proto;
        if (!x.stream) HIP_CHECK(hipStreamCreateWithFlags(&x.stream, hipStreamNonBlocking));
        x.work.reserve(frame_work_bytes(dims) + (ahead ? frame_ahead_bytes(dims) : 0)); x.cls.reserve(ahead ? pad256(cls_bytes) + cls_bytes : cls_bytes);
        uint8_t *w = x.work.ptr, *c = x.cls.ptr;
        place_frame(f, dims, tiles_x, w, c);
        const uint32_t* cost_before = x.strip_cost.ptr;
        x.strip_cost.reserve(dims.strip_cost_count());
        if (x.strip_cost.ptr != cost_before) HIP_CHECK(hipMemsetAsync(x.strip_cost.ptr, 0, x.strip_cost.cap * sizeof(uint32_t), up_stream));
        f.strip_cost = x.strip_cost.ptr;
        r->d_counters.reserve(8 * COUNTER_WORDS);
        f.counters = x.counters = r->d_counters.ptr + size_t(k) * COUNTER_WORDS;
        HIP_CHECK(hipMemsetAsync(x.cls.ptr, 0, ahead ? pad256(cls_bytes) + cls_bytes : cls_bytes, up_stream));
        if (!x.d_fb.ptr && !r->n_targets) {
            x.d_fb.reserve(size_t(r->width) * r->height);
            HIP_CHECK(hipMemsetAsync(x.d_fb.ptr, 0, size_t(r->width) * r->height * 4, up_stream));
        }
        f.fb = (fb_override && k == si) ? fb_override : (r->n_targets ? r->targets[uint32_t(k) % r->n_targets] : x.d_fb.ptr);
        if (ahead) {
            Frame2& f1 = fr[4 + k];
            f1 = f;
            place_frame_ahead(f1, dims, tiles_x, w, c);
            const uint32_t* cost1_before = x.strip_cost_ahead.ptr;
            x.strip_cost_ahead.reserve(dims.strip_cost_count());
            if (x.strip_cost_ahead.ptr != cost1_before) HIP_CHECK(hipMemsetAsync(x.strip_cost_ahead.ptr, 0, x.strip_cost_ahead.cap * sizeof(uint32_t), up_stream));
            f1.strip_cost = x.strip_cost_ahead.ptr;
            f1.counters = r->d_counters.ptr + size_t(4 + k) * COUNTER_WORDS;
        }
    }
    sc.frames_dev = static_cast<Frame2*>(A.push(fr, sizeof fr));
    sc.frames_ahead = ahead ? sc.frames_dev + 4 : nullptr;
    A.flush(up_stream, si == 0);
    if (all_sets) {
        for (int k = 0; k < n_sets; ++k)
            if (k != si && r->fs[k].stream) HIP_CHECK(hipStreamWaitEvent(r->fs[k].stream, A.copied, 0));
    }
    if (r->bitmap_table_dirty) {
        if (!r->bitmap_table.empty())
            HIP_CHECK(hipMemcpyAsync(r->d_bitmap_table.ptr, r->bitmap_table.data(), r->bitmap_table.size() * sizeof(DevBitmap),
                                     hipMemcpyHostToDevice, r->stream));
        r->bitmap_table_dirty = false;
        r->bitmap_table_dirty_copied = true;
    }
    if (r->bitmap_table_dirty_copied) { HIP_CHECK(hipStreamSynchronize(r->stream)); r->bitmap_table_dirty_copied = false; }
    if (si == 0) { r->scene_ready = true; r->sets_ready = all_sets ? uint32_t(n_sets) : 1u; r->scene_from_builder = edges_tagged; ++r->scene_gen; }
    return SWFR_OK;
}

void validate_linear_pixman(const swfr_renderer* r, const SceneView& sv) {
    const auto [edges, n_edges, paths, n_paths, styles, n_styles] = sv;
    bool any = false;
    for (size_t i = 0; i < n_styles; ++i) any = any || styles[i].kind >= SWFR_STYLE_LINEAR_PIXMAN;
    if (!any) return;
    for (size_t i = 0; i < n_styles; ++i) {
        const swfr_style& s = styles[i];
        if (s.kind > SWFR_STYLE_LINEAR_PIXMAN) throw StatusError{SWFR_ERR_INVALID, "unknown style kind"};
        if (s.kind != SWFR_STYLE_LINEAR_PIXMAN) continue;
        if (r->mono) throw StatusError{SWFR_ERR_NOT_IMPLEMENTED, "NotImplementedAliasedPixmanLinear"};
        if (s.n_stops > SWFR_MAX_STOPS) throw StatusError{SWFR_ERR_INVALID, "too many gradient stops"};
        if (s.c0x == s.c1x && s.c0y == s.c1y) throw StatusError{SWFR_ERR_INVALID, "a pixman-linear gradient needs two distinct points (c0 == c1)"};
        if (s.c0x != -16384.0 || s.c0y != 0.0 || s.c1x != 16384.0 || s.c1y != 0.0) throw StatusError{SWFR_ERR_NOT_IMPLEMENTED, "NotImplementedLinearLine"};
    }
    for (size_t i = 0; i < n_paths; ++i) {
        const swfr_path& p = paths[i];
        if (size_t(p.first_edge) + p.n_edges > n_edges || (p.kind < SWFR_PATH_GROUP_BEGIN && p.style >= n_styles) || p.kind > SWFR_PATH_GROUP_MASK) return;
        if (p.x_min < 0 || p.y_min < 0 || p.x_max > int(r->width) || p.y_max > int(r->height) || p.x_min > p.x_max || p.y_min > p.y_max) return;
    }
    std::vector<DevFilter> filters; std::vector<DevGradient> gradients; std::vector<int32_t> fparams; size_t n_linear = 0;
    std::vector<swfr_style> only;
    only.assign(styles, styles + n_styles);
    for (swfr_style& s : only) if (s.kind != SWFR_STYLE_LINEAR_PIXMAN) { s.kind = SWFR_STYLE_SOLID; }
    std::vector<swfr_path> drawn;
    for (size_t i = 0; i < n_paths; ++i) if (paths[i].kind < SWFR_PATH_GROUP_BEGIN) drawn.push_back(paths[i]);
    prepare_sources(SceneView{edges, n_edges, drawn.data(), drawn.size(), only.data(), n_styles}, false, n_linear, filters, gradients, fparams, r->bitmap_table, r->variant_table, r->blur_table);
}

void validate_upload(const swfr_renderer* r, const SceneView& sv) {
    const bool alpha_modes = (r->cfg.flags & SWFR_FLAG_ALPHA_MODES) != 0;
    validate_groups(sv, alpha_modes);
    validate_blend_fields(sv, alpha_modes);
    validate_gradient_extend(sv);
    validate_bitmap_filter(sv);
    validate_linear_pixman(r, sv);
    if (!r->has_device) throw StatusError{SWFR_ERR_NO_DEVICE, "host-only handle cannot rasterize"};
    validate_scene(r, sv);
}

void launch_chain(swfr_renderer* r, hipStream_t st, const Frame2* frames, uint32_t n_frames, const LaunchPlan& p, hipEvent_t* events, uint32_t* fb_to) {
    if (events) HIP_CHECK(hipEventRecord(events[0], st));
    r->last_bin_threads = p.bin_threads;
    launch2_bin(st, frames, n_frames, p.max_edges, p.max_paths, p.max_bands, p.slow_kernels, r->mono, p.bin_threads);
    if (events) HIP_CHECK(hipEventRecord(events[1], st));
    launch2_rows(st, frames, n_frames, p.max_chunks, p.max_path_edges, p.rows_wide, r->mono);
    if (p.run_slow) launch2_rows_slow(st, frames, n_frames, p.grid_slow, p.grid_huge, p.slow_passes, r->mono);
    launch2_linear_pieces(st, frames, n_frames, p.linear_grid);
    if (events) HIP_CHECK(hipEventRecord(events[2], st));
    launch2_tiles(st, frames, n_frames, p.max_strips, p.tiles_grid, p.shader_level, fb_to);
    if (events) HIP_CHECK(hipEventRecord(events[3], st));
}
uint32_t bin_threads_of(const swfr_renderer* r, uint32_t max_paths, bool overlapped) {
    if (r->bin_threads) return uint32_t(r->bin_threads);
    return overlapped && max_paths <= BIN_SMALL_PATHS ? BIN_THREADS_SMALL : BIN_THREADS_LARGE;
}
LaunchPlan plan_of(const swfr_renderer* r, const swfr_renderer::Scene& sc) {
    LaunchPlan p = sc.bounds;
    p.run_slow = p.max_chunks && sc.slow_state != 1;
    p.slow_kernels = p.run_slow ? 1u : 0u;
    p.bin_threads = bin_threads_of(r, p.max_paths, true);
    p.grid_slow = 1024u; p.grid_huge = sc.slow_state == 2 ? 0u : 256u; p.slow_passes = sc.slow_passes;
    p.tiles_grid = r->tiles_grid > 0 ? uint32_t(r->tiles_grid) : ~0u;
    return p;
}

void launch_frame(swfr_renderer* r, const swfr_renderer::Scene& sc, swfr_renderer::FrameSet& F, uint32_t* fb, hipEvent_t* e, bool overlapped) {
// ... 81 lines not shown
}
void release_bitmap_slot(swfr_renderer* r, uint32_t id, DeviceBitmap& slot) {
    if (slot.pixels) HIP_CHECK(hipFree(slot.pixels));
    if (slot.d_straight) HIP_CHECK(hipFree(slot.d_straight));
    if (slot.straight_ready) HIP_CHECK(hipEventDestroy(slot.straight_ready));
    slot = DeviceBitmap{};
    for (auto it = r->cx_cache.begin(); it != r->cx_cache.end();) {
        if (it->second.bitmap == id && !it->second.pinned) {
            cx_quiesce(r);
            (void)hipFree(it->second.pixels);
            if (it->second.ready) (void)hipEventDestroy(it->second.ready);
            r->cx_bytes -= it->second.bytes;
            it = r->cx_cache.erase(it);
        } else ++it;
    }
}

int render_resident(swfr_renderer* r, uint32_t frames) {
    if (!r->has_device) return fail(r, SWFR_ERR_NO_DEVICE, "host-only handle cannot rasterize");
    if (!r->scene_ready) return fail(r, SWFR_ERR_INVALID, "no scene uploaded");
    if (frames == 0) frames = 1;
    if (frames > 1 && r->scene_from_builder && r->sets_ready < uint32_t(std::max(1, std::min(r->in_flight, 4)))) {
        const int rc = upload2(r, 0, true, builder_view(r), nullptr, true);
        if (rc != SWFR_OK) return rc;
    }
    if (frames > 1 && r->use_graphs && !r->scn[0].slow_verified) {
        const int rc = render_resident(r, 1);
        if (rc != SWFR_OK) return rc;
        --frames;
    }
    const swfr_renderer::Scene& sc = r->scn[0];
    float setup_ms = 0, rows_ms = 0, tiles_ms = 0, total_ms = 0;
    uint32_t counters[COUNTER_WORDS] = {};
    if (frames > 4096) frames = 4096;
    uint32_t n_sets = 1;
    if (frames > 1)
        while (n_sets < uint32_t(std::min(r->in_flight, 4)) && n_sets < r->sets_ready && r->fs[n_sets].stream && (r->n_targets || r->fs[n_sets].d_fb.ptr)) ++n_sets;
    uint32_t stride = r->event_stride < 1 ? 1u : uint32_t(r->event_stride);
    if (frames < 64 && !r->event_stride_given) stride = std::min(stride, 8u);
    const uint32_t first_timed = std::min(stride / 2, frames - 1);
    const uint32_t n_timed = (frames - first_timed + stride - 1) / stride;
    while (r->ev.size() < size_t(n_timed) * 4 + 5) {
        hipEvent_t e = nullptr;
        HIP_CHECK(hipEventCreate(&e));
        r->ev.push_back(e);
    }
    hipEvent_t ev_begin = r->ev[size_t(n_timed) * 4], ev_end = r->ev[size_t(n_timed) * 4 + 1];
    hipEvent_t* ev_join = &r->ev[size_t(n_timed) * 4 + 2];
    if (frames > 1 && r->use_graphs && sc.slow_verified && !(r->resident_batch >= 2 && stride > frames))
        for (uint32_t k = 0; k < n_sets; ++k) ensure_frame_graph(r, sc, r->fs[k]);
    HIP_CHECK(hipEventRecord(ev_begin, r->stream));
    order_frames_behind_pending_read(r);
#ifdef SWFR_BEGIN_WAIT
    for (uint32_t k = 1; k < n_sets; ++k) HIP_CHECK(hipStreamWaitEvent(r->fs[k].stream, ev_begin, 0));
#endif
    uint32_t rb = (r->resident_batch >= 2 && stride > frames) ? uint32_t(r->resident_batch) : 1u;
    while (rb > 1 && (rb > n_sets || n_sets % rb != 0)) --rb;
    const bool batched = rb > 1 && frames >= 2;
    uint32_t last_set = (frames - 1) % n_sets;
    int64_t last_on[4] = {-1, -1, -1, -1};
    uint32_t last_parity[4] = {0, 0, 0, 0};
    r->last_ahead_launches = 0;
    if (batched) {
        const uint32_t groups = n_sets / rb;
        const LaunchPlan plan = plan_of(r, sc);
        const bool ahead = r->bin_ahead && sc.frames_ahead && sc.slow_verified && !plan.run_slow && !plan.linear_grid && !r->mono && !r->bin_threads &&
                           !r->use_graphs && !rows_wide_instance(plan.max_path_edges, plan.rows_wide);
        const uint32_t launches = (frames + rb - 1) / rb;
        uint32_t gi = 0;
        for (uint32_t f = 0; f < frames; f += rb, ++gi) {
            const uint32_t g = gi % groups, cnt = std::min(rb, frames - f);
            const hipStream_t st = r->fs[g * rb].stream;
            if (!ahead) launch_chain(r, st, sc.frames_dev + g * rb, cnt, plan, nullptr, nullptr);
            else {
                const uint32_t parity = (gi / groups) & 1u;
                const Frame2* cur = (parity ? sc.frames_ahead : sc.frames_dev) + g * rb;
                const Frame2* next = (parity ? sc.frames_dev : sc.frames_ahead) + g * rb;
                if (gi < groups) {
                    r->last_bin_threads = plan.bin_threads;
                    launch2_bin(st, cur, cnt, plan.max_edges, plan.max_paths, plan.max_bands, 0u, false, plan.bin_threads);
                }
                if (gi + groups < launches) {
                    const uint32_t next_cnt = std::min(rb, frames - (f + groups * rb));
                    launch2_rows_ahead(st, cur, next, cnt, next_cnt, plan.max_edges, plan.max_paths, plan.max_bands, plan.max_chunks);
                    ++r->last_ahead_launches;
                } else launch2_rows(st, cur, cnt, plan.max_chunks, plan.max_path_edges, false, false);
                launch2_tiles(st, cur, cnt, plan.max_strips, plan.tiles_grid, plan.shader_level, nullptr);
                for (uint32_t k = 0; k < cnt; ++k) last_parity[g * rb + k] = parity;
            }
            last_set = g * rb + cnt - 1;
            last_on[g * rb] = int64_t(gi);
        }
    }
    for (uint32_t f = 0; f < frames && !batched; ++f) {
        swfr_renderer::FrameSet& F = r->fs[f % n_sets];
        const bool timed = f >= first_timed && (f - first_timed) % stride == 0;
        if (!timed && frames > 1 && r->use_graphs && sc.slow_verified) launch_frame_graph(r, sc, F);
        else launch_frame(r, sc, F, nullptr, timed ? &r->ev[size_t((f - first_timed) / stride) * 4] : nullptr, n_sets > 1 && frames > 1);
        last_on[f % n_sets] = int64_t(f);
    }
    for (uint32_t k = 1; k < n_sets; ++k) {
        if (last_on[k] < 0) continue;
        HIP_CHECK(hipEventRecord(ev_join[k - 1], r->fs[k].stream));
        HIP_CHECK(hipStreamWaitEvent(r->stream, ev_join[k - 1], 0));
    }
    HIP_CHECK(hipEventRecord(ev_end, r->stream));
    HIP_CHECK(hipGetLastError());
    if (!r->h_counters) HIP_CHECK(hipHostMalloc(reinterpret_cast<void**>(&r->h_counters), 8 * COUNTER_WORDS * sizeof(uint32_t), hipHostMallocDefault));
    const uint32_t used_sets = std::min(frames, n_sets);
    const bool any_ahead = r->last_ahead_launches != 0;
    HIP_CHECK(hipMemcpyAsync(r->h_counters, r->d_counters.ptr, size_t(any_ahead ? 8 : used_sets) * COUNTER_WORDS * sizeof(uint32_t), hipMemcpyDeviceToHost, r->stream));
    for (;;) {
        int pick = -1;
        for (uint32_t k = 1; k < n_sets; ++k)
            if (last_on[k] >= 0 && (pick < 0 || last_on[k] < last_on[pick])) pick = int(k);
        if (pick < 0) break;
        if (r->fs[pick].stream) HIP_CHECK(hipStreamSynchronize(r->fs[pick].stream));
        last_on[pick] = -1;
    }
    HIP_CHECK(hipStreamSynchronize(r->stream));
    r->fb_cur = r->n_targets ? r->targets[last_set % r->n_targets] : r->fs[last_set].d_fb.ptr;
    uint32_t timed_frames = 0;
    for (uint32_t f = batched ? frames : first_timed; f < frames; f += stride, ++timed_frames) {
        hipEvent_t* e = &r->ev[size_t(timed_frames) * 4];
        float a = 0, b = 0, c = 0;
        HIP_CHECK(hipEventElapsedTime(&a, e[0], e[1]));
        HIP_CHECK(hipEventElapsedTime(&b, e[1], e[2]));
        HIP_CHECK(hipEventElapsedTime(&c, e[2], e[3]));
        setup_ms += a; rows_ms += b; tiles_ms += c;
    }
    HIP_CHECK(hipEventElapsedTime(&total_ms, ev_begin, ev_end));
    for (uint32_t k = 0; k < used_sets; ++k)
        if (last_parity[k]) std::memcpy(r->h_counters + k * COUNTER_WORDS, r->h_counters + (4 + k) * COUNTER_WORDS, COUNTER_WORDS * sizeof(uint32_t));
    std::memcpy(counters, r->h_counters, sizeof counters);
    for (uint32_t k = 1; k < used_sets; ++k)
        for (uint32_t w : {uint32_t(C2_ERROR), uint32_t(C2_TIE_PAIRTEST_SKIPPED), uint32_t(C2_TIE_SORT_OVERFLOW), uint32_t(C2_TIE_DEPTH)})
            counters[w] |= r->h_counters[k * COUNTER_WORDS + w];
    r->timing = swfr_timing{total_ms, setup_ms, rows_ms, tiles_ms, frames, sc.dims.n_edges, sc.dims.n_paths, sc.dims.n_rows, 0, timed_frames};
    r->fb_valid = true;
    {
        uint32_t slow = 0, huge = 0;
        for (uint32_t k = 0; k < used_sets; ++k) { slow |= r->h_counters[k * COUNTER_WORDS + C2_SLOW]; huge |= r->h_counters[k * COUNTER_WORDS + C2_HUGE]; }
        uint32_t passes = 1;
        for (uint32_t k = 0; k < used_sets; ++k)
            for (uint32_t q = 1; q < SLOW_PASSES; ++q) {
                const uint32_t* c = r->h_counters + k * COUNTER_WORDS;
                if (c[C2_SLOWQ + q] | c[C2_HUGEQ + q]) { passes = std::max(passes, q + 1); huge |= c[C2_HUGEQ + q]; }
            }
        const bool short_launch = (sc.slow_state == 1 && slow) || (sc.slow_state == 2 && huge) || passes > sc.slow_passes;
        r->scn[0].slow_state = slow == 0 ? 1 : (huge == 0 ? 2 : 0);
        r->scn[0].slow_passes = passes;
        r->hint_slow_state = r->scn[0].slow_state; r->hint_slow_passes = passes;
        r->scn[0].slow_verified = !short_launch;
        if (short_launch) {
            r->scn[0].slow_state = 0; r->scn[0].slow_passes = SLOW_PASSES;
            r->fb_valid = false;
            return render_resident(r, frames);
        }
        r->timing.n_records = 0;
        for (uint32_t h = 0; h < C2_HEADS; ++h) r->timing.n_records += counters[C2_HEAD + h];
    }
    return check_counters(r, counters);
}

int render_blur_layers(swfr_renderer* r) {
    const auto& layers = r->builder->layers();
    if (r->cfg.band_count > 1) throw StatusError{SWFR_ERR_NOT_IMPLEMENTED, "NotImplementedBlurBands"};
// ... 299 lines not shown
    if (r->h_image_cap < bytes) {
        if (r->h_image) (void)hipHostFree(r->h_image);
        r->h_image = nullptr; r->h_image_cap = 0;
        HIP_CHECK(hipHostMalloc(reinterpret_cast<void**>(&r->h_image), bytes, hipHostMallocDefault));
        r->h_image_cap = bytes;
    }
    if (!r->read_done) HIP_CHECK(hipEventCreateWithFlags(&r->read_done, hipEventDisableTiming));
    HIP_CHECK(hipMemcpyAsync(r->h_image, src, bytes, hipMemcpyDeviceToHost, r->stream));
    HIP_CHECK(hipEventRecord(r->read_done, r->stream));
    r->read_pending = true;
    return SWFR_OK;
}
int finish_read(swfr_renderer* r) {
    if (!r->read_pending) return fail(r, SWFR_ERR_INVALID, "no read-back in flight");
    HIP_CHECK(hipEventSynchronize(r->read_done));
    r->read_pending = false;
    return SWFR_OK;
}

int render_resident_async(swfr_renderer* r, void* block_target, uint32_t* out_set) {
    if (!r->has_device) return fail(r, SWFR_ERR_NO_DEVICE, "host-only handle cannot rasterize");
    if (!r->scene_ready) return fail(r, SWFR_ERR_INVALID, "no scene uploaded");
    const BandShare bs = band_share(r);
    if (block_target && bs.stride != 1) return fail(r, SWFR_ERR_INVALID, "a block target needs a handle that owns one contiguous block of tile-rows");
    return guarded(r, [&]() {
        uint32_t n_sets = 1;
        while (n_sets < uint32_t(std::min(r->in_flight, 4)) && n_sets < r->sets_ready && r->fs[n_sets].stream && r->fs[n_sets].work.ptr) ++n_sets;
        const uint32_t k = r->async_next++ % n_sets;
        r->async_used |= 1u << k;
        if (!r->scn[0].slow_verified) { r->scn[0].slow_state = 0; r->scn[0].slow_passes = SLOW_PASSES; }
        uint32_t* fb_to = block_target ? static_cast<uint32_t*>(block_target) - size_t(bs.first) * TILE_H * r->width : nullptr;
        order_frames_behind_pending_read(r);
        launch_frame(r, r->scn[0], r->fs[k], fb_to, nullptr, block_target || n_sets > 1);
        HIP_CHECK(hipGetLastError());
        r->fb_cur = block_target ? nullptr : (r->n_targets ? r->targets[k % r->n_targets] : r->fs[k].d_fb.ptr);
        if (block_target) r->fb_valid = false;
        if (out_set) *out_set = k;
        return int(SWFR_OK);
    });
}

thread_local const char* create_error = nullptr;

}

extern "C" {
#pragma GCC visibility push(default)

uint32_t swfr_abi_version(void) { return SWFR_ABI_VERSION; }

const char* swfr_last_error(const swfr_renderer* r) { return r ? r->error.c_str() : (create_error ? create_error : "null handle"); }

int swfr_create(uint32_t width, uint32_t height, const swfr_config* cfg, swfr_renderer** out) {
    if (!out) return SWFR_ERR_INVALID;
    *out = nullptr;
    if (width == 0 || height == 0 || width > 32768 || height > 32768) return SWFR_ERR_INVALID;
    std::unique_ptr<swfr_renderer> r(new (std::nothrow) swfr_renderer);
    if (!r) return SWFR_ERR_CAPACITY;
    r->width = width;
    r->height = height;
    if (cfg) r->cfg = *cfg;
    if (r->cfg.band_count > 1 && r->cfg.band_index >= r->cfg.band_count) return SWFR_ERR_INVALID;
    r->mono = (r->cfg.flags & SWFR_FLAG_ANTIALIAS_NONE) != 0;
    create_error = nullptr;
    if (r->mono && (r->cfg.flags & SWFR_FLAG_LINEAR_PIXMAN)) { create_error = "NotImplementedAliasedPixmanLinear"; return SWFR_ERR_NOT_IMPLEMENTED; }
    r->builder.reset(new FrameBuilder(width, height, (r->cfg.flags & SWFR_FLAG_EVEN_ODD) != 0, r->mono, (r->cfg.flags & SWFR_FLAG_LINEAR_PIXMAN) != 0,
                                        (r->cfg.flags & SWFR_FLAG_ALPHA_MODES) != 0));
    if (const char* fl = std::getenv("SWFR_FAST_LIMIT")) r->fast_limit = std::atoi(fl);
    if (const char* tg = std::getenv("SWFR_TILES_GRID")) r->tiles_grid = std::atoi(tg);
    if (const char* bt = std::getenv("SWFR_BIN_THREADS")) { const int v = std::atoi(bt); r->bin_threads = v == int(BIN_THREADS_SMALL) || v == int(BIN_THREADS_LARGE) ? v : 0; }
    if (const char* ts = std::getenv("SWFR_TILES_SHADERS")) r->tiles_shaders = std::min(std::max(std::atoi(ts), 0), 7);
    if (const char* rw = std::getenv("SWFR_ROWS_WIDE")) r->rows_wide = std::atoi(rw) != 0;
    if (const char* bf = std::getenv("SWFR_BATCH_FRAMES")) r->batch_frames = std::max(1, std::atoi(bf));
    if (const char* cr = std::getenv("SWFR_CHUNK_ROWS")) r->force_chunk_rows = std::atoi(cr);
    if (const char* so = std::getenv("SWFR_STRIP_ORDER")) r->strip_order = std::atoi(so);
    if (const char* fi = std::getenv("SWFR_FRAMES_IN_FLIGHT")) r->in_flight = std::atoi(fi);
    if (const char* es = std::getenv("SWFR_EVENT_STRIDE")) { r->event_stride = std::atoi(es); r->event_stride_given = true; }
    if (const char* ug = std::getenv("SWFR_GRAPHS")) r->use_graphs = std::atoi(ug);
#ifdef SWFR_EMU
    r->use_graphs = 0;
#endif
    if (const char* rb = std::getenv("SWFR_RESIDENT_BATCH")) r->resident_batch = std::atoi(rb);
    if (const char* ba = std::getenv("SWFR_BIN_AHEAD")) r->bin_ahead = std::atoi(ba) != 0;
    if (const char* cm = std::getenv("SWFR_CXFORM_CACHE_MB")) r->cx_budget = size_t(std::max(0, std::atoi(cm))) << 20;
    if (r->cfg.device == SWFR_DEVICE_HOST_ONLY) {
        *out = r.release();
        return SWFR_OK;
    }
    int count = 0;
    if (hipGetDeviceCount(&count) != hipSuccess || count <= 0) return SWFR_ERR_NO_DEVICE;
    if (r->cfg.device < 0 || r->cfg.device >= count) return SWFR_ERR_NO_DEVICE;
    r->has_device = true;
    swfr_renderer* raw = r.get();
    const int rc = guarded(raw, [&]() {
        HIP_CHECK(hipStreamCreateWithFlags(&raw->stream, hipStreamNonBlocking));
        raw->fs[0].stream = raw->stream;
        for (int k = 1; k < std::max(1, std::min(raw->in_flight, 4)); ++k) HIP_CHECK(hipStreamCreateWithFlags(&raw->fs[k].stream, hipStreamNonBlocking));
        for (int i = 0; i < 4 * 32 + 5; ++i) { hipEvent_t e = nullptr; HIP_CHECK(hipEventCreate(&e)); raw->ev.push_back(e); }
        raw->fs[0].d_fb.reserve(size_t(width) * height);
        HIP_CHECK(hipMemsetAsync(raw->fs[0].d_fb.ptr, 0, size_t(width) * height * 4, raw->stream));
        raw->d_counters.reserve(8 * COUNTER_WORDS);
        raw->fs[0].counters = raw->d_counters.ptr;
        HIP_CHECK(hipStreamSynchronize(raw->stream));
        return int(SWFR_OK);
    });
    if (rc != SWFR_OK) return rc;
    *out = r.release();
    return SWFR_OK;
}

void swfr_destroy(swfr_renderer* r) { delete r; }

int swfr_register_shape(swfr_renderer* r, const swfr_define_shape* tag, uint32_t* out_id) {
    if (!r || !tag || !out_id) return fail(r, SWFR_ERR_INVALID, "null argument");
    return guarded(r, [&]() {
        *out_id = r->builder->add_shape(decode_shape(*tag, false));
        return int(SWFR_OK);
    });
}

int swfr_register_morph_shape(swfr_renderer* r, const swfr_define_shape* tag, uint32_t* out_id) {
    if (!r || !tag || !out_id) return fail(r, SWFR_ERR_INVALID, "null argument");
    return guarded(r, [&]() {
        *out_id = r->builder->add_morph_shape(decode_shape(*tag, true));
        return int(SWFR_OK);
    });
}

int swfr_decode_x_swf_bmp(const uint8_t* data, size_t len, uint32_t* width, uint32_t* height, uint8_t* rgba, size_t rgba_cap) {
    if (!data || !width || !height) return SWFR_ERR_INVALID;
    try {
        std::vector<uint8_t> px;
        const XSwfBmpStatus st = decode_x_swf_bmp(data, len, *width, *height, px);
        if (st == XSwfBmpStatus::UnsupportedFormat) return SWFR_ERR_NOT_IMPLEMENTED;
        if (st != XSwfBmpStatus::Ok) return SWFR_ERR_INVALID;
        if (rgba) {
            if (rgba_cap < px.size()) return SWFR_ERR_CAPACITY;
            std::memcpy(rgba, px.data(), px.size());
        }
        return SWFR_OK;
    } catch (...) { return SWFR_ERR_DEVICE; }
}

int swfr_register_bitmap_tag(swfr_renderer* r, uint32_t id, const char* media_type, const uint8_t* data, size_t len) {
    if (!r || !media_type || !data) return fail(r, SWFR_ERR_INVALID, "null argument");
    if (std::strcmp(media_type, "image/x-swf-bmp") != 0)
        return fail(r, SWFR_ERR_NOT_IMPLEMENTED, std::string("NotImplemented: Support for ") + media_type + " images");
    uint32_t w = 0, h = 0;
    std::vector<uint8_t> px;
    XSwfBmpStatus st = XSwfBmpStatus::Corrupt;
    try { st = decode_x_swf_bmp(data, len, w, h, px); } catch (...) { return fail(r, SWFR_ERR_DEVICE, "out of memory decoding a bitmap"); }
    if (st == XSwfBmpStatus::UnsupportedFormat) return fail(r, SWFR_ERR_NOT_IMPLEMENTED, std::string("UnsupportedXSwfBmpFormatId: ") + std::to_string(len ? int(data[0]) : -1));
    if (st != XSwfBmpStatus::Ok) return fail(r, SWFR_ERR_INVALID, "corrupt image/x-swf-bmp data");
    return swfr_register_bitmap(r, id, w, h, px.data(), size_t(w) * 4);
}

int swfr_register_bitmap(swfr_renderer* r, uint32_t id, uint32_t width, uint32_t height, const uint8_t* rgba, size_t stride) {
    if (!r || !rgba || width == 0 || height == 0 || stride < size_t(width) * 4) return fail(r, SWFR_ERR_INVALID, "bad bitmap");
    if (id > 65535) return fail(r, SWFR_ERR_INVALID, "bitmap id out of range");
    return guarded(r, [&]() {
        r->builder->add_bitmap(id, BitmapInfo{width, height});
        if (!r->has_device) return int(SWFR_OK);
        std::vector<uint32_t> argb(size_t(width) * height);
        for (uint32_t y = 0; y < height; ++y) {
            const uint8_t* row = rgba + size_t(y) * stride;
            for (uint32_t x = 0; x < width; ++x) {
// ... 568 lines not shown
```

### swf_renderer_amd/csrc/rows3.hip

```cpp

#if defined(R3_MARKS) && !defined(SWFR_EMU)
#define R3MARK(n) asm volatile("; R3MARK " #n)
#else
#define R3MARK(n) do { } while (0)
#endif
template <int STAGE> struct R3Mask { typedef uint32_t type; };
template <> struct R3Mask<64> { typedef uint64_t type; };
__device__ __forceinline__ int r3_first(uint32_t m) { return __ffs((int)m) - 1; }
__device__ __forceinline__ int r3_first(uint64_t m) { return __ffsll((long long)m) - 1; }
__device__ __forceinline__ int r3_count(uint32_t m) { return __popc(m); }
__device__ __forceinline__ int r3_count(uint64_t m) { return __popcll(m); }

__device__ __forceinline__ uint32_t lane_bit(uint64_t m, int lane) {
#ifdef SWFR_EMU
    return (uint32_t)((m >> lane) & 1ull);
#else
    (void)lane;
    uint32_t r;
    asm("v_cndmask_b32_e64 %0, 0, 1, %1" : "=v"(r) : "s"(m));
    return r;
#endif
}
__device__ __forceinline__ uint32_t cols_from(int u) { return u >= 32 ? 0u : (u <= 0 ? ~0u : (~0u << u)); }
__device__ __forceinline__ uint32_t col_bit(int t) { return (uint32_t)t < 32u ? (1u << t) : 0u; }

#define R3_BIAS (1 << 24)
#define R3_INVALID(s) (0xF0000000u | ((uint32_t)(s) << 5) | (uint32_t)(s))
#define R3_KEY(c, dir, s) ((((uint32_t)((c) + R3_BIAS)) << 5) | ((dir) > 0 ? 16u : 0u) | (uint32_t)(s))
#define R3_PAST(s, nm) ((((s) & 1) == 0) && (s) >= (nm))
#define R3_CE(i, j) do { const uint32_t lo_ = min(key[i], key[j]), hi_ = max(key[i], key[j]); key[i] = lo_; key[j] = hi_; } while (0)
#define R3_CEP(i, j) do { const bool sw_ = key[i] > key[j]; const uint32_t lo_ = min(key[i], key[j]), hi_ = max(key[i], key[j]); \
                          const int a_ = sw_ ? c1[j] : c1[i], b_ = sw_ ? c1[i] : c1[j]; key[i] = lo_; key[j] = hi_; c1[i] = a_; c1[j] = b_; } while (0)
#define R3_NET4(CE) do { CE(0, 1); CE(2, 3); CE(0, 2); CE(1, 3); CE(1, 2); } while (0)
#define R3_NET6(CE) do { CE(1, 2); CE(4, 5); CE(0, 2); CE(3, 5); CE(0, 1); CE(3, 4); CE(2, 5); CE(0, 3); CE(1, 4); CE(2, 4); CE(1, 3); CE(2, 3); } while (0)
#define R3_NET16(CE) do { CE(0, 1); CE(2, 3); CE(0, 2); CE(1, 3); CE(1, 2); CE(4, 5); CE(6, 7); CE(4, 6); CE(5, 7); CE(5, 6); CE(0, 4); CE(2, 6); CE(2, 4); CE(1, 5); CE(3, 7); CE(3, 5); CE(1, 2); CE(3, 4); CE(5, 6); CE(8, 9); CE(10, 11); CE(8, 10); CE(9, 11); CE(9, 10); CE(12, 13); CE(14, 15); CE(12, 14); CE(13, 15); CE(13, 14); CE(8, 12); CE(10, 14); CE(10, 12); CE(9, 13); CE(11, 15); CE(11, 13); CE(9, 10); CE(11, 12); CE(13, 14); CE(0, 8); CE(4, 12); CE(4, 8); CE(2, 10); CE(6, 14); CE(6, 10); CE(2, 4); CE(6, 8); CE(10, 12); CE(1, 9); CE(5, 13); CE(5, 9); CE(3, 11); CE(7, 15); CE(7, 11); CE(3, 5); CE(7, 9); CE(11, 13); CE(1, 2); CE(3, 4); CE(5, 6); CE(7, 8); CE(9, 10); CE(11, 12); CE(13, 14); } while (0)
#define R3_NET8(CE) do { CE(0, 1); CE(2, 3); CE(4, 5); CE(6, 7); CE(0, 2); CE(1, 3); CE(4, 6); CE(5, 7); CE(1, 2); CE(5, 6); CE(0, 4); CE(3, 7); \
                         CE(1, 5); CE(2, 6); CE(1, 4); CE(3, 6); CE(2, 4); CE(3, 5); CE(3, 4); } while (0)

__device__ __forceinline__ void full_cells3(int32_t qt, int32_t qb, int32_t rl, int32_t DX, int32_t D, double invW, int32_t fq0, double fr0, int neg,
                                            int xminp, int xmaxp, Cell* __restrict__ dst) {
    int ix1 = qt >> 8, f1 = qt & 255, ix2 = qb >> 8, f2 = qb & 255;
    if (ix1 == ix2) { put_cell_h(dst, ix1, (15 ^ neg) - neg, f1 + f2, xminp, xmaxp); return; }
    int32_t ql = qt;
    if (ix2 < ix1) { int t = ix1; ix1 = ix2; ix2 = t; t = f1; f1 = f2; f2 = t; ql = qb; }
    const int span = ix2 - ix1 + 1;
    const double W = 512.0 * fabs((double)DX);
    const double num = fma((double)((ix1 + 1) * 256 - ql), (double)D, -(double)rl);
    double yqf = floor(num * invW);
    double yr = fma(-yqf, W, num);
    if (yr < 0.0) { yqf -= 1.0; yr += W; }
    if (yr >= W) { yqf += 1.0; yr -= W; }
    int yq = (int)yqf;
    int y_prev = yq;
    if (span <= MAX_CELLS_PER_EDGE_ROW) {
        put_cell_h(dst, ix1, (y_prev ^ neg) - neg, 256 + f1, xminp, xmaxp);
#pragma unroll 1
        for (int k = 1; k < span - 1; ++k) {
            yq += fq0; yr += fr0; if (yr >= W) { ++yq; yr -= W; }
            put_cell_h(dst + k, ix1 + k, ((yq - y_prev) ^ neg) - neg, 256, xminp, xmaxp);
            y_prev = yq;
        }
        put_cell_h(dst + span - 1, ix2, ((15 - y_prev) ^ neg) - neg, f2, xminp, xmaxp);
        return;
    }
    int n = 0;
    if (y_prev) put_cell_h(dst + n++, ix1, (y_prev ^ neg) - neg, 256 + f1, xminp, xmaxp);
#pragma unroll 1
    for (int c = ix1 + 1; c < ix2; ++c) {
        yq += fq0; yr += fr0; if (yr >= W) { ++yq; yr -= W; }
        const int h = yq - y_prev;
        if (h && n < MAX_CELLS_PER_EDGE_ROW - 1) put_cell_h(dst + n++, c, (h ^ neg) - neg, 256, xminp, xmaxp);
        y_prev = yq;
    }
    if (15 - y_prev) put_cell_h(dst + n++, ix2, ((15 - y_prev) ^ neg) - neg, f2, xminp, xmaxp);
    while (n < MAX_CELLS_PER_EDGE_ROW) put_cell(dst + n++, xminp, 0, 0, xminp, xmaxp);
}

template <int STAGE, int NS>
__device__ __forceinline__ void rows3_chunk_body(FramePtr FR, uint32_t block) {
    typedef typename R3Mask<STAGE>::type amask_t;
    __shared__ __attribute__((aligned(16))) FastEdge staged[STAGE];
    __shared__ __attribute__((aligned(16))) uint32_t sub_cells[4][NS * 15];
    __shared__ uint32_t sub_masks[4][4];
    __shared__ uint8_t slot_role[NS][64];
    __shared__ uint8_t slot_edge[NS][64];
    __shared__ uint32_t mid_bits[2];
    TRACE_DECL;
    TRACE_NOWAIT(0);
    const int lane = threadIdx.x;
    const ChunkInfo ck = FR->chunks[block];
    const uint32_t lo = ck.path;
    const FastEdge* __restrict__ FE = fast_edges_of(FR->edges, FR->n_edges) + ck.first_edge;
    const FastEdge ek_first = FE[min((uint32_t)lane, ck.n_edges ? ck.n_edges - 1u : 0u)];
    const DevPath P = FR->paths[lo];
    const int r = (int)ck.first_row + lane;
    const int chunk_rows = (int)ck.rows;

    const int g16 = (((int)ck.first_row & (TILE_H - 1)) + lane) >> 4;
    const int band = (int)ck.first_row / TILE_H + g16;
    const int band_lo = P.y_min / TILE_H, band_hi = (P.y_max - 1) / TILE_H;
    BandSlot cls_bs = {0u, 0u, 0u, 0u};
    uint32_t cls_b0 = 0, cls_b1 = 0;
    if (ck.slot0 != ~0u && lane < chunk_rows) {
        cls_bs = FR->band_slots[ck.slot0 + (uint32_t)g16];
        const uint32_t bclamp = min((uint32_t)band, FR->n_bands - 1u);
        cls_b0 = FR->band_off[bclamp];
        cls_b1 = FR->band_off[bclamp + 1u];
    }
    const bool band_ok = ck.slot0 != ~0u && lane < chunk_rows && band >= band_lo && band <= band_hi && P.kind == SWFR_PATH_TOR;
    const uint32_t ri = band_ok ? cls_bs.slot * TILE_H + (uint32_t)(r & (TILE_H - 1)) : ~0u;
    const bool in_path = P.kind == SWFR_PATH_TOR && lane < chunk_rows && r >= P.y_min && r < P.y_max;
    bool live = in_path;
    { uint32_t lb; if (live && !owns_band(FR, r / TILE_H, lb)) live = false; }
    if (__ballot(live) == 0ull) {
        if (ri != ~0u && lane < chunk_rows) { RowInfo2 h; h.off = 0; h.n = 0; h.mode = (uint16_t)(in_path ? (uint32_t)ROW_FOREIGN : (uint32_t)ROW_EMPTY); FR->rows[ri] = h; }
        return;
    }
    TRACE(1);
    R3MARK(1);
    SWFR_GLOBAL_PTR(Cell) p_cells = (SWFR_GLOBAL_PTR(Cell))FR->cells; SWFR_GLOBAL_PTR(RowInfo2) p_rows = (SWFR_GLOBAL_PTR(RowInfo2))FR->rows;
#define R3_FIELD(name) ((decltype(FR->name))p_##name)
    const int fast_limit = min((int)FR->fast_limit, NS);
    const int lo_s = (int)ck.first_row * 15, hi_s = lo_s + chunk_rows * 15;
    if (lane < 2) mid_bits[lane] = 0u;
    uint32_t n_list = 0;
    bool use_lds = true;
    int inc_before = 0;
    for (uint32_t eb = 0; eb < ck.n_edges; eb += 64) {
        const uint32_t k = eb + (uint32_t)lane;
        const FastEdge ek = eb == 0 ? ek_first : FE[min(k, ck.n_edges - 1u)];
        const bool valid = k < ck.n_edges && ek.ybot > ek.ytop;
        if (valid) inc_before += max(0, min((ek.ybot - 1) / 15 + 1, (int)ck.first_row) - ek.ytop / 15);
        const bool hit = use_lds && valid && ek.ytop < hi_s && ek.ybot > lo_s;
        const unsigned long long hb = __ballot(hit);
        const uint32_t at = n_list + (uint32_t)__popcll(hb & ((1ull << lane) - 1ull));
        if (hit && at < (uint32_t)STAGE) staged[at] = ek;
        n_list += (uint32_t)__popcll(hb);
        if (n_list > (uint32_t)STAGE) use_lds = false;
    }
    const uint32_t chunk_cell_base = (ck.rec_base + (uint32_t)__builtin_amdgcn_readlane(wave_scan_incl(inc_before), 63)) * (uint32_t)MAX_CELLS_PER_EDGE_ROW;
    bool forced_over = false;
    if (!use_lds) {
        int cnt = 0;
        for (uint32_t k = 0; k < P.n_edges; ++k) {
            const int yt = FE[k].ytop, yb = FE[k].ybot;
            if (yb > r * 15 && yt < r * 15 + 15) ++cnt;
        }
        const bool fast_row = live && cnt > 0 && cnt <= fast_limit;
        const unsigned long long fm = __ballot(fast_row);
        forced_over = live && cnt > 0 && !fast_row;
        n_list = 0;
        bool ok = fm != 0ull;
        lds_barrier();
        for (uint32_t eb = 0; ok && eb < P.n_edges; eb += 64) {
            const uint32_t k = eb + (uint32_t)lane;
            const FastEdge ek = FE[min(k, P.n_edges - 1u)];
            const int ra = ek.ytop / 15 - (int)ck.first_row, rz = (ek.ybot + 14) / 15 - (int)ck.first_row;
            const int a = min(max(ra, 0), 64), b = min(max(rz, 0), 64);
            const uint64_t bits = (b >= 64 ? ~0ull : ((1ull << b) - 1ull)) & ~(a >= 64 ? ~0ull : ((1ull << a) - 1ull));
            const bool hit = k < P.n_edges && ek.ybot > ek.ytop && (bits & fm) != 0ull;
            const unsigned long long hb = __ballot(hit);
            const uint32_t at = n_list + (uint32_t)__popcll(hb & ((1ull << lane) - 1ull));
            if (hit && at < (uint32_t)STAGE) staged[at] = ek;
            n_list += (uint32_t)__popcll(hb);
            if (n_list > (uint32_t)STAGE) ok = false;
        }
        use_lds = ok;
        if (!ok) { n_list = 0; forced_over = live && cnt > 0; }
    }
    lds_barrier();
    SWFR_PIN_SGPR(p_cells); SWFR_PIN_SGPR(p_rows);
    R3MARK(2);
    uint32_t rb_lo = 0, rb_hi = 0;
    if (use_lds && (uint32_t)lane < n_list) {
        const int yt = staged[lane].ytop, yb = staged[lane].ybot;
        const int ra = yt / 15 - (int)ck.first_row, rz = (yb + 14) / 15 - (int)ck.first_row;
        const int a = min(max(ra, 0), 64), b = min(max(rz, 0), 64);
        const uint64_t below_b = b >= 64 ? ~0ull : ((1ull << b) - 1ull), below_a = a >= 64 ? ~0ull : ((1ull << a) - 1ull);
        const uint64_t bits = below_b & ~below_a;
        rb_lo = (uint32_t)bits; rb_hi = (uint32_t)(bits >> 32);
        uint64_t mb = 0;
        if (yt % 15 != 0 && ra >= 0 && ra < 64) mb |= 1ull << ra;
        if (yb % 15 != 0 && rz >= 1 && rz <= 64) mb |= 1ull << (rz - 1);
        if ((uint32_t)mb) atomicOr(&mid_bits[0], (uint32_t)mb);
        if ((uint32_t)(mb >> 32)) atomicOr(&mid_bits[1], (uint32_t)(mb >> 32));
    }
    lds_barrier();
    TRACE(2);
    R3MARK(3);
    amask_t amask = 0;
    if (use_lds)
        for (int k = (int)n_list - 1; k >= 0; --k) {
            const uint64_t m = ((uint64_t)(uint32_t)__builtin_amdgcn_readlane((int)rb_hi, k) << 32) | (uint64_t)(uint32_t)__builtin_amdgcn_readlane((int)rb_lo, k);
            amask = (amask_t)(amask << 1) | (amask_t)lane_bit(m, lane);
        }
    const uint64_t mid_mask = ((uint64_t)(uint32_t)__builtin_amdgcn_readfirstlane((int)mid_bits[1]) << 32) | (uint64_t)(uint32_t)__builtin_amdgcn_readfirstlane((int)mid_bits[0]);
    const bool mid_row = lane_bit(mid_mask, lane) != 0u;
    if (!live) amask = 0;
    int n = r3_count(amask);
    const bool overflow = live && (forced_over || n > fast_limit);
    if (overflow) { n = 0; amask = 0; }
    const int nmax = (NS > 8 && __ballot(n > 8)) ? 16 : __ballot(n > 6) ? 8 : __ballot(n > 4) ? 6 : __ballot(n > 2) ? 4 : 2;
    const int s0 = r * 15;
    const unsigned fmask = P.fill_rule ? 1u : ~0u;

    R3MARK(4);
    uint32_t key[NS]; int c1[NS];
    int32_t qt[NS], qb[NS], rl[NS];
#ifdef ABL3_NOEVAL
    const bool can_full = false;
#else
    const bool can_full = n > 0 && !mid_row;
#endif
    {
        amask_t m = amask;
#pragma unroll
        for (int s = 0; s < NS; ++s) {
            if (R3_PAST(s, nmax)) break;
            key[s] = R3_INVALID(s); c1[s] = 0x7fffffff;
            const int k = m ? r3_first(m) : 0;
            m &= m - 1;
            slot_edge[s][lane] = (uint8_t)k;
            const FastEdge& e = staged[k];
            const int32_t x1 = e.x1, DX = e.DX, D = e.D, hD = D >> 1;
            int32_t q, rm;
            fast_x_at(e.a0, DX, D, e.invD, s0, q, rm);
            const int32_t xa = x1 + q;
            const int c0 = xa + (rm >= hD ? 1 : 0);
            int32_t xb = xa + e.q15, rn = rm + e.r15;
            if (rn >= D) { ++xb; rn -= D; }
            const int c1v = xb + (rn >= hD ? 1 : 0);
            const int32_t hq = e.hq, hr = e.hr;
            int32_t qa = xa - hq, ra = rm - hr; if (ra < 0) { --qa; ra += D; }
            int32_t qz = xb - hq, rz = rn - hr; if (rz < 0) { --qz; rz += D; }
            const bool valid = can_full && s < n;
            if (valid) { key[s] = R3_KEY(c0, e.dir, s); c1[s] = c1v; }
            qt[s] = qa; qb[s] = qz; rl[s] = DX < 0 ? rz : ra;
        }
    }
    TRACE(3);
    R3MARK(5);
    if (nmax <= 2) R3_CEP(0, 1);
    else if (nmax <= 4) R3_NET4(R3_CEP);
    else if (nmax <= 6) R3_NET6(R3_CEP);
    else if (nmax <= 8) R3_NET8(R3_CEP);
    else if constexpr (NS > 8) R3_NET16(R3_CEP);
    bool full = can_full, deep = false;
    unsigned tie_bits = 0;
#pragma unroll
    for (int p = 0; p + 1 < NS; ++p) {
        if (R3_PAST(p + 1, nmax)) break;
        if (c1[p] > c1[p + 1]) full = false;
        if ((key[p] >> 5) == (key[p + 1] >> 5)) { tie_bits |= 1u << p; deep = true; }
    }
    bool defer = false;
    if (__ballot(deep && can_full) != 0ull) {
        if (deep && can_full) {
            bool real = false;
#pragma unroll
            for (int p = 0; p + 1 < NS; ++p) {
                if (R3_PAST(p + 1, nmax)) break;
                if ((tie_bits >> p) & 1u) {
                    const FastEdge& ea = staged[slot_edge[key[p] & 15u][lane]];
                    const FastEdge& eb = staged[slot_edge[key[p + 1] & 15u][lane]];
                    real |= !(ea.x1 == eb.x1 && ea.a0 == eb.a0 && ea.DX == eb.DX && ea.D == eb.D);
                }
            }
            defer = real;
        }
    }
    uint32_t mode = ROW_EMPTY;
    bool is_sub = false;
    uint32_t roles = 0;
#define R3_ROLE(s) ((roles >> (2 * (s))) & 3u)
    if (n > 0) {
        if (defer) mode = ROW_DEFER;
        else if (full) mode = ROW_FULL;
        else { mode = ROW_SUB; is_sub = true; }
    }
// ... 176 lines not shown
        a_and &= (uint32_t)__builtin_amdgcn_update_dpp(0, (int)a_and, 0x128, 0xf, 0xf, false);
        a_or |= (uint32_t)__builtin_amdgcn_update_dpp(0, (int)a_or, 0x128, 0xf, 0xf, false);
        a_int |= (uint32_t)__builtin_amdgcn_update_dpp(0, (int)a_int, 0x128, 0xf, 0xf, false);
        a_and &= (uint32_t)__builtin_amdgcn_update_dpp(0, (int)a_and, 0x124, 0xf, 0xf, false);
        a_or |= (uint32_t)__builtin_amdgcn_update_dpp(0, (int)a_or, 0x124, 0xf, 0xf, false);
        a_int |= (uint32_t)__builtin_amdgcn_update_dpp(0, (int)a_int, 0x124, 0xf, 0xf, false);
        a_and &= (uint32_t)__builtin_amdgcn_update_dpp(0, (int)a_and, 0x122, 0xf, 0xf, false);
        a_or |= (uint32_t)__builtin_amdgcn_update_dpp(0, (int)a_or, 0x122, 0xf, 0xf, false);
        a_int |= (uint32_t)__builtin_amdgcn_update_dpp(0, (int)a_int, 0x122, 0xf, 0xf, false);
        a_and &= (uint32_t)__builtin_amdgcn_update_dpp(0, (int)a_and, 0x121, 0xf, 0xf, false);
        a_or |= (uint32_t)__builtin_amdgcn_update_dpp(0, (int)a_or, 0x121, 0xf, 0xf, false);
        a_int |= (uint32_t)__builtin_amdgcn_update_dpp(0, (int)a_int, 0x121, 0xf, 0xf, false);
        if (sub == 0 && R >= 0) { sub_masks[g][0] = a_int; sub_masks[g][1] = a_and; sub_masks[g][2] = a_or; }
        lds_barrier();
        {
            const int my_t = (int)__builtin_amdgcn_mbcnt_hi((uint32_t)(pass_rows >> 32), __builtin_amdgcn_mbcnt_lo((uint32_t)pass_rows, 0u));
            if (lane_bit(pass_rows, lane) != 0u) { m_inter = sub_masks[my_t][0]; m_and = sub_masks[my_t][1]; m_or = sub_masks[my_t][2]; }
        }
        {
            const uint32_t c0 = (uint32_t)__builtin_amdgcn_readlane((int)n_merged, 15), c1r = (uint32_t)__builtin_amdgcn_readlane((int)n_merged, 31);
            const uint32_t c2 = (uint32_t)__builtin_amdgcn_readlane((int)n_merged, 47), c3 = (uint32_t)__builtin_amdgcn_readlane((int)n_merged, 63);
            const uint32_t total = c0 + c1r + c2 + c3;
            const uint32_t b0 = (uint32_t)__builtin_amdgcn_readlane((int)my_room, Rs[0]), b1 = (uint32_t)__builtin_amdgcn_readlane((int)my_room, Rs[1]);
            const uint32_t b2 = (uint32_t)__builtin_amdgcn_readlane((int)my_room, Rs[2]), b3 = (uint32_t)__builtin_amdgcn_readlane((int)my_room, Rs[3]);
            for (uint32_t t = (uint32_t)lane; t < total; t += 64) {
                const int gg = t < c0 ? 0 : (t < c0 + c1r ? 1 : (t < c0 + c1r + c2 ? 2 : 3));
                const uint32_t pre = gg == 0 ? 0u : (gg == 1 ? c0 : (gg == 2 ? c0 + c1r : c0 + c1r + c2));
                const uint32_t bb = gg == 0 ? b0 : (gg == 1 ? b1 : (gg == 2 ? b2 : b3));
                const uint32_t w = sub_cells[gg][t - pre];
                sub_cells[gg][t - pre] = 0u;
                const uint32_t v = (uint32_t)((int)(w << 13) >> 13);
                if (wave_base != ~0u) R3_FIELD(cells)[bb + (t - pre)] = Cell{(w - v) | (v & 0x7ffffu)};
            }
            if (sub == 0 && R >= 0 && riR != ~0u) {
                const uint32_t bb = g == 0 ? b0 : (g == 1 ? b1 : (g == 2 ? b2 : b3));
                const uint32_t cg = g == 0 ? c0 : (g == 1 ? c1r : (g == 2 ? c2 : c3));
                RowInfo2 h; h.off = wave_base == ~0u ? 0u : bb; h.n = wave_base == ~0u ? (uint16_t)0 : (uint16_t)cg; h.mode = (uint16_t)ROW_SUB;
                R3_FIELD(rows)[riR] = h;
            }
        }
        lds_barrier();
    }
    TRACE(5);
    R3MARK(10);
    const bool slow = live && (overflow || defer);
    if (ri != ~0u && lane < chunk_rows && mode != ROW_SUB) {
        RowInfo2 h; h.off = 0; h.n = 0; h.mode = (uint16_t)(slow ? (uint32_t)ROW_DEFER : (in_path && !live) ? (uint32_t)ROW_FOREIGN : mode);
        if (mode == ROW_FULL && !slow && wave_base != ~0u) { h.off = my_room; h.n = (uint16_t)n_cells; }
        R3_FIELD(rows)[ri] = h;
    }
    {
        const bool q = slow && ri != ~0u;
        const unsigned long long qm = __ballot(q);
        if (qm) {
            uint32_t qbase = 0;
            if (lane == 0) {
                qbase = atomicAdd(&FR->counters[C2_SLOW], (uint32_t)__popcll(qm));
                if (atomicOr(&FR->path_flag[lo], 1u) == 0u) FR->path_queue[atomicAdd(&FR->counters[C2_PATHQ], 1u)] = lo;
            }
            qbase = (uint32_t)__builtin_amdgcn_readfirstlane((int)qbase);
            if (q) {
                const uint32_t at = qbase + (uint32_t)__popcll(qm & ((1ull << lane) - 1ull));
                if (at < FR->slow_cap) {
                    SlowRow sr; sr.path = lo; sr.row = r; sr.ri = ri;
                    sr.pad = (ck.slot0 - (uint32_t)((int)ck.first_row / TILE_H - band_lo)) | (defer ? 0x80000000u : 0u);
                    FR->slow[at] = sr;
                }
                else atomicOr(&FR->counters[C2_ERROR], E2_SLOW_QUEUE);
            }
        }
    }
    R3MARK(11);
#ifdef ABL3_NOCLASS
    if (ck.slot0 == 0x7ffffff0u)
#endif
    if (ck.slot0 != ~0u && P.kind == SWFR_PATH_TOR) {
        const int width = FR->width, height = FR->height;
        uint8_t* out = FR->cls;
        uint32_t n_b = 0;
        if (band_ok) {
            n_b = cls_b1 - cls_b0;
            out = FR->cls + (size_t)STRIPS_PER_TILE * FR->tiles_x * cls_b0 + (cls_bs.slot - cls_b0);
        }
        const swfr_style& st = style_at(FR, P.style);
        const uint32_t opq = (st.kind == SWFR_STYLE_SOLID && P.lerp && (st.pixel >> 24) == 0xffu) ? CLS_OPAQUE : 0u;
        const bool in_frame = r < height && band_ok, in_rows = in_frame && in_path;
        uint32_t local_trow = 0;
        const bool own_band = band_ok && owns_band(FR, band, local_trow);
        const bool cost_order = FR->strip_order != 0u;
        const uint32_t pos1 = cls_bs.slot - cls_b0 + 1u;
        const int strip_in_tile = (r >> 3) & 1, tsub = lane & 7;
        for (int tb = 0; tb < ntc; tb += 32) {
            const int nb = min(ntc - tb, 32);
            const uint32_t colmask = nb >= 32 ? ~0u : ((1u << nb) - 1u);
            uint32_t iv = m_inter, cand = m_and, cor = m_or;
            if (tb > 0) {
                iv = 0; cand = 0; cor = 0;
                if (mode == ROW_FULL) { uint32_t i2, c2; full_row_masks(tc0 + tb, i2, c2); iv = i2; cand = c2; cor = c2; }
                else if (mode == ROW_SUB) iv = ~0u;
            }
            uint32_t inside = colmask;
            if (tb == 0 && P.x_min > tc0 * TILE_W) inside &= ~1u;
            if (tb + nb == ntc && P.x_max < min((tc1 + 1) * TILE_W, width)) inside &= ~(1u << (nb - 1));
            uint32_t mp = 0, mn = 0, me = 0, mh = 0;
            if (in_frame) {
                if (!in_rows) mn = colmask;
                else if (slow) { mp = mn = me = colmask; }
                else {
                    iv &= colmask; cand &= colmask; cor &= colmask;
                    mp = iv | (cor & ~cand) | (cand & ~inside);
                    me = iv | cor;
                    mh = colmask & ~me;
                    mn = mp | mh;
                }
            }
            const unsigned long long pb = __ballot(in_rows && (slow || (iv & colmask) != 0u));
#define R3_OR8(v) do { v |= (uint32_t)__builtin_amdgcn_update_dpp(0, (int)v, 0x141, 0xf, 0xf, false); \
                       v |= (uint32_t)__builtin_amdgcn_update_dpp(0, (int)v, 0xb1, 0xf, 0xf, false); \
                       v |= (uint32_t)__builtin_amdgcn_update_dpp(0, (int)v, 0x4e, 0xf, 0xf, false); } while (0)
            R3_OR8(mp); R3_OR8(mn); R3_OR8(me); R3_OR8(mh);
#undef R3_OR8
            mp |= mh & me;
            for (int t0 = 0; t0 < nb; t0 += 8) {
                const int t = t0 + tsub;
                uint32_t f = (((mp >> t) & 1u) ? CLS_PARTIAL : 0u) | (((mn >> t) & 1u) ? CLS_NOTFULL : 0u) | (((me >> t) & 1u) ? CLS_NONEMPTY : 0u);
                if (f == CLS_NONEMPTY) f |= opq;
                const int tc = tc0 + tb + t;
                if (t < nb && band_ok && lane < chunk_rows) {
                    out[(uint32_t)(tc * STRIPS_PER_TILE + strip_in_tile) * n_b] = (uint8_t)f;
                    if (own_band) {
                        const uint32_t strip_id = (local_trow * (uint32_t)FR->tiles_x + (uint32_t)tc) * STRIPS_PER_TILE + (uint32_t)strip_in_tile;
                        strip_top_note(FR, strip_id, pos1, f, st.pixel);
                        if (cost_order && (f & CLS_PARTIAL)) {
                            const uint32_t wgt = (uint32_t)__popcll((pb >> (lane & ~7)) & 0xffull);
                            if (wgt) atomicAdd(&FR->strip_cost[strip_id], wgt);
                        }
                    }
                }
            }
        }
    }
#undef R3_FIELD
    TRACE(7);
    TRACE_OUT(1, block);
}
```

Measured before the change: 408,200.

## Precompute per-chunk edge lists in the ahead bin pass for the rows kernel

Adds a StageRec per chunk. The look-ahead binning blocks of the next frame fill it with the chunk's overlapping edge indices, row masks, mid-row bits, the cell-base increment, the path rectangle/flags and band offsets. The rows kernel can then load this record and skip its own edge scan, ballot compaction, path load and band_off lookups. The goal is to move that per-chunk setup into the overlapped ahead work. In exchange it adds extra global memory per frame set, serial per-lane edge loops in the bin pass, and a runtime toggle that defaults to off.

```diff
diff --git a/swf_renderer_amd/csrc/device_types.hpp b/swf_renderer_amd/csrc/device_types.hpp
--- a/swf_renderer_amd/csrc/device_types.hpp
+++ b/swf_renderer_amd/csrc/device_types.hpp
@@ -1,5 +1,6 @@
 #pragma once
 
+#include <stddef.h>
 #include <stdint.h>
 
 #include "../../include/swfr.h"
@@ -55,6 +56,24 @@
     uint32_t first_edge, n_edges;
     uint32_t pad;
 };
+
+constexpr uint32_t STAGE_REC_EDGES = 32;
+constexpr uint32_t STAGE_REC_NONE = ~0u;
+struct StageRec {
+    uint32_t n_list;
+    uint32_t inc_before;
+    uint32_t mid_lo, mid_hi;
+    int32_t x_min, x_max, y_min, y_max;
+    uint32_t flags;
+    uint32_t pixel;
+    uint32_t pad0[2];
+    uint32_t band_off[4][2];
+    uint8_t idx[STAGE_REC_EDGES];
+    uint32_t pad1[4];
+    uint64_t mask[STAGE_REC_EDGES];
+};
+static_assert(sizeof(StageRec) == 384 && offsetof(StageRec, idx) == 80 && offsetof(StageRec, mask) == 128, "StageRec layout");
+enum : uint32_t { STAGE_REC_FILL_RULE = 1u, STAGE_REC_TOR = 2u, STAGE_REC_OPAQUE = 4u };
 
 struct BandSlot {
     uint32_t path;
diff --git a/swf_renderer_amd/csrc/frame_layout.hpp b/swf_renderer_amd/csrc/frame_layout.hpp
--- a/swf_renderer_amd/csrc/frame_layout.hpp
+++ b/swf_renderer_amd/csrc/frame_layout.hpp
@@ -62,6 +62,12 @@
     return bytes;
 }
 
+inline size_t stage_rec_bytes(const FrameDims& d) { return pad256(d.chunk_count() * sizeof(StageRec)); }
+inline uint8_t* carve_stage_recs(StageRec*& p, const FrameDims& d, uint8_t* base) {
+    p = reinterpret_cast<StageRec*>(base);
+    return base + stage_rec_bytes(d);
+}
+
 inline size_t cls_bytes_of(size_t n_slots, size_t tiles_x) { return (size_t(STRIPS_PER_TILE) * n_slots * tiles_x + 64 + 15) & ~size_t(15); }
 inline size_t cls_region_bytes(size_t n_slots, size_t tiles_x, size_t n_strips) { return cls_bytes_of(n_slots, tiles_x) + (n_strips + 1) * sizeof(StripTop); }
 inline size_t cls_region_bytes(const FrameDims& d, size_t tiles_x) { return cls_region_bytes(d.n_slots, tiles_x, d.n_strips); }
diff --git a/swf_renderer_amd/csrc/raster2.hip b/swf_renderer_amd/csrc/raster2.hip
--- a/swf_renderer_amd/csrc/raster2.hip
+++ b/swf_renderer_amd/csrc/raster2.hip
@@ -162,7 +162,7 @@
 #ifndef BIN_ORDER_FIRST_LARGE
 #define BIN_ORDER_FIRST_LARGE 0
 #endif
-template <uint32_t BIN_THREADS, bool ORDER_FIRST> __device__ __forceinline__ void bin_body(FramePtr F, uint32_t slow_kernels) {
+template <uint32_t BIN_THREADS, bool ORDER_FIRST, bool STAGE_AHEAD = false> __device__ __forceinline__ void bin_body(FramePtr F, uint32_t slow_kernels, StageRec* __restrict__ stage = nullptr) {
     constexpr uint32_t BAND_LIST = 4 * BIN_THREADS;
     static_assert(BIN_THREADS % 64 == 0 && BIN_THREADS >= (uint32_t)C2_WORDS, "whole wavefronts; block 0 clears the counters in one step");
     __shared__ uint32_t wave_cnt[BIN_THREADS / 64];
@@ -310,6 +310,81 @@
         const uint32_t b_fe = (uint32_t)__shfl((int)first_edge, src), b_ne = (uint32_t)__shfl((int)n_path_edges, src), b_band0 = (uint32_t)__shfl((int)band0, src);
         for (uint32_t c = (uint32_t)lane; c < b_nc; c += 64u) write_chunk(b_path, c, b_a0, b_c0, b_inc0, b_slots0, b_fe, b_ne, b_band0);
     }
+    if constexpr (STAGE_AHEAD) {
+        if (stage == nullptr) return;
+        SWFR_GLOBAL_PTR(StageRec) stg = (SWFR_GLOBAL_PTR(StageRec))stage;
+        const int rows = (int)F->chunk_rows;
+        const uint32_t n_bands = F->n_bands, cap = F->chunk_cap;
+        auto stage_edge = [&](SWFR_GLOBAL_PTR(StageRec) rec, int first_row, uint32_t k, int yt, int yb, uint32_t& cnt, uint32_t& inc, uint64_t& mid) {
+            inc += (uint32_t)max(0, min((yb - 1) / 15 + 1, first_row) - yt / 15);
+            if (!(yt < (first_row + rows) * 15 && yb > first_row * 15)) return;
+            if (cnt < STAGE_REC_EDGES) {
+                const int ra = yt / 15 - first_row, rz = (yb + 14) / 15 - first_row;
+                const int a = min(max(ra, 0), 64), b = min(max(rz, 0), 64);
+                const uint64_t below_b = b >= 64 ? ~0ull : ((1ull << b) - 1ull), below_a = a >= 64 ? ~0ull : ((1ull << a) - 1ull);
+                rec->idx[cnt] = (uint8_t)k;
+                rec->mask[cnt] = below_b & ~below_a;
+                if (yt % 15 != 0 && ra >= 0 && ra < 64) mid |= 1ull << ra;
+                if (yb % 15 != 0 && rz >= 1 && rz <= 64) mid |= 1ull << (rz - 1);
+            }
+            ++cnt;
+        };
+        auto stage_header = [&](SWFR_GLOBAL_PTR(StageRec) rec, const DevPath& P, int first_row, uint32_t cnt, uint32_t inc, uint64_t mid) {
+            const uint32_t kind = style_at(F, P.style).kind, pixel = style_at(F, P.style).pixel;
+            rec->n_list = (cnt <= STAGE_REC_EDGES && P.n_edges <= 256u) ? cnt : STAGE_REC_NONE; rec->inc_before = inc; rec->mid_lo = (uint32_t)mid; rec->mid_hi = (uint32_t)(mid >> 32);
+            rec->x_min = P.x_min; rec->x_max = P.x_max; rec->y_min = P.y_min; rec->y_max = P.y_max;
+            rec->flags = (P.fill_rule ? STAGE_REC_FILL_RULE : 0u) | (P.kind == SWFR_PATH_TOR ? STAGE_REC_TOR : 0u) |
+                         ((kind == SWFR_STYLE_SOLID && P.lerp && (pixel >> 24) == 0xffu) ? STAGE_REC_OPAQUE : 0u);
+            rec->pixel = pixel; rec->pad0[0] = 0; rec->pad0[1] = 0;
+#pragma unroll
+            for (int t = 0; t < 4; ++t) {
+                const uint32_t bclamp = min((uint32_t)(first_row / TILE_H + t), n_bands - 1u);
+                rec->band_off[t][0] = F->band_off[bclamp]; rec->band_off[t][1] = F->band_off[bclamp + 1u];
+            }
+        };
+        {
+            constexpr uint32_t STAGE_PASS = 4;
+            const bool own = nc != 0u && nc <= OWN_CHUNKS;
+            DevPath P = {};
+            if (own) P = F->paths[ip];
+            const uint32_t ne = own ? n_path_edges : 0u, n_own = own ? nc : 0u;
+            for (uint32_t cb = 0; cb < n_own; cb += STAGE_PASS) {
+                uint32_t cnt[STAGE_PASS], inc[STAGE_PASS]; uint64_t mid[STAGE_PASS];
+#pragma unroll
+                for (uint32_t j = 0; j < STAGE_PASS; ++j) { cnt[j] = 0; inc[j] = 0; mid[j] = 0; }
+                for (uint32_t k = 0; k < ne; ++k) {
+                    int32_t yt, yb;
+                    fast_edge_span(F->raw[first_edge + k], P, yt, yb);
+                    if (yb <= yt) continue;
+#pragma unroll
+                    for (uint32_t j = 0; j < STAGE_PASS; ++j)
+                        if (cb + j < nc && c0 + cb + j < cap) stage_edge(stg + (c0 + cb + j), (int)(a0 + (cb + j) * (uint32_t)rows), k, yt, yb, cnt[j], inc[j], mid[j]);
+                }
+#pragma unroll
+                for (uint32_t j = 0; j < STAGE_PASS; ++j)
+                    if (cb + j < nc && c0 + cb + j < cap) stage_header(stg + (c0 + cb + j), P, (int)(a0 + (cb + j) * (uint32_t)rows), cnt[j], inc[j], mid[j]);
+            }
+        }
+        for (unsigned long long big = __ballot(nc > OWN_CHUNKS); big; big &= big - 1ull) {
+            const int src = __ffsll((long long)big) - 1;
+            const uint32_t b_nc = (uint32_t)__shfl((int)nc, src), b_path = (uint32_t)__shfl((int)ip, src), b_a0 = (uint32_t)__shfl((int)a0, src);
+            const uint32_t b_c0 = (uint32_t)__shfl((int)c0, src), b_fe = (uint32_t)__shfl((int)first_edge, src), b_ne = (uint32_t)__shfl((int)n_path_edges, src);
+            const DevPath P = F->paths[b_path];
+            for (uint32_t cb = 0; cb < b_nc; cb += 64u) {
+                const uint32_t c = cb + (uint32_t)lane;
+                const bool mine = c < b_nc && b_c0 + c < cap;
+                SWFR_GLOBAL_PTR(StageRec) rec = stg + (mine ? b_c0 + c : b_c0);
+                const int first_row = (int)(b_a0 + c * (uint32_t)rows);
+                uint32_t cnt = 0, inc = 0; uint64_t mid = 0;
+                for (uint32_t k = 0; k < b_ne; ++k) {
+                    int32_t yt, yb;
+                    fast_edge_span(F->raw[b_fe + k], P, yt, yb);
+                    if (yb > yt && mine) stage_edge(rec, first_row, k, yt, yb, cnt, inc, mid);
+                }
+                if (mine) stage_header(rec, P, first_row, cnt, inc, mid);
+            }
+        }
+    }
 }
 constexpr uint32_t ORDER_RANGES = 8;
 __device__ __forceinline__ uint32_t order_range(uint32_t cost) {
@@ -439,18 +514,19 @@
     if (blockIdx.x >= FR->n_chunks) return;
     rows3_chunk_body<ROWS_STAGE_WIDE, ROWS_FAST_WIDE>(FR, blockIdx.x);
 }
-__global__ __launch_bounds__(64) R2_ATTR void k2_rows_ahead_b(const Frame2* __restrict__ frames, const Frame2* __restrict__ ahead, uint32_t n_ahead, uint32_t ahead_frames) {
+__global__ __launch_bounds__(64) R2_ATTR void k2_rows_ahead_b(const Frame2* __restrict__ frames, const Frame2* __restrict__ ahead, uint32_t n_ahead, uint32_t ahead_frames,
+                                                              StageRec* const* __restrict__ stage_frames, StageRec* const* __restrict__ stage_ahead) {
     if (blockIdx.x < n_ahead) {
         if (blockIdx.y >= ahead_frames) return;
         TRACE_DECL; TRACE_NOWAIT(0);
-        bin_body<BIN_THREADS_AHEAD, true>(FRAME_PTR(ahead, blockIdx.y), 0u);
+        bin_body<BIN_THREADS_AHEAD, true, true>(FRAME_PTR(ahead, blockIdx.y), 0u, stage_ahead ? stage_ahead[blockIdx.y] : nullptr);
         TRACE(7); TRACE_OUT(0, blockIdx.x);
         return;
     }
     FramePtr FR = FRAME_PTR(frames, blockIdx.y);
     const uint32_t chunk = blockIdx.x - n_ahead;
     if (chunk >= FR->n_chunks) return;
-    rows3_chunk_body<ROWS_STAGE, ROWS_FAST_N>(FR, chunk);
+    rows3_chunk_body<ROWS_STAGE, ROWS_FAST_N, true>(FR, chunk, stage_frames ? stage_frames[blockIdx.y] : nullptr);
 }
 
 #include "mono.hip"
@@ -1802,10 +1878,11 @@
     if (rows_wide_instance(max_path_edges, wide)) hipLaunchKernelGGL(k2_rows_wide_b, dim3(max_chunks, n_frames), dim3(64), 0, st, frames);
     else hipLaunchKernelGGL(k2_rows_b, dim3(max_chunks, n_frames), dim3(64), 0, st, frames);
 }
-void launch2_rows_ahead(hipStream_t st, const Frame2* frames, const Frame2* ahead, uint32_t n_frames, uint32_t ahead_frames, uint32_t max_edges, uint32_t max_paths, uint32_t max_bands, uint32_t max_chunks) {
+void launch2_rows_ahead(hipStream_t st, const Frame2* frames, const Frame2* ahead, uint32_t n_frames, uint32_t ahead_frames, uint32_t max_edges, uint32_t max_paths, uint32_t max_bands, uint32_t max_chunks,
+                        StageRec* const* stage_frames, StageRec* const* stage_ahead) {
     constexpr uint32_t T = BIN_THREADS_AHEAD;
     const uint32_t n_ahead = XCDS + max_bands + (max_edges + T - 1) / T + (max_paths + T - 1) / T;
-    hipLaunchKernelGGL(k2_rows_ahead_b, dim3(n_ahead + max_chunks, n_frames), dim3(64), 0, st, frames, ahead, n_ahead, ahead_frames);
+    hipLaunchKernelGGL(k2_rows_ahead_b, dim3(n_ahead + max_chunks, n_frames), dim3(64), 0, st, frames, ahead, n_ahead, ahead_frames, stage_frames, stage_ahead);
 }
 void launch2_rows_slow(hipStream_t st, const Frame2* frames, uint32_t n_frames, uint32_t grid_slow, uint32_t grid_huge, uint32_t max_passes, bool mono) {
     if (mono) { hipLaunchKernelGGL(k2_rows_mono_huge_b, dim3(grid_huge ? grid_huge : 64u, n_frames), dim3(HUGE_THREADS), 0, st, frames); return; }
diff --git a/swf_renderer_amd/csrc/raster_common.hip b/swf_renderer_amd/csrc/raster_common.hip
--- a/swf_renderer_amd/csrc/raster_common.hip
+++ b/swf_renderer_amd/csrc/raster_common.hip
@@ -4,6 +4,7 @@
 #ifdef SWFR_EMU
 #include <cstdio>
 #include <cstdlib>
+#include <cstring>
 #endif
 
 #include "device_types.hpp"
@@ -139,16 +140,21 @@
     return d;
 }
 
+__device__ __forceinline__ void edge_span_clamped(const swfr_edge& e, const DevPath& p, int32_t& ytop_out, int32_t& ybot_out) {
+    int ytop = (int)((15ll * e.top + 128) >> 8), ybot = (int)((15ll * e.bottom + 128) >> 8);
+    ytop = max(ytop, p.y_min * 15);
+    ybot = min(ybot, p.y_max * 15);
+    if (ybot <= ytop) { ytop = ybot = 0; }
+    ytop_out = ytop; ybot_out = ybot;
+}
+__device__ __forceinline__ void fast_edge_span(const swfr_edge& e, const DevPath& p, int32_t& ytop, int32_t& ybot) {
+    edge_span_clamped(e, p, ytop, ybot);
+    if (p.kind != SWFR_PATH_TOR || e.y2 <= e.y1) ytop = ybot = 0;
+}
 __device__ __forceinline__ FastEdge make_fast_edge(const swfr_edge& e, const DevPath& p) {
     FastEdge f;
     f.x1 = e.x1; f.a0 = 256 - 30 * e.y1; f.DX = 0; f.D = 30; f.invD = 1.0 / 30.0; f.q15 = f.r15 = f.hq = f.hr = f.dqf = f.drf = 0;
-    {
-        int ytop = (int)((15ll * e.top + 128) >> 8), ybot = (int)((15ll * e.bottom + 128) >> 8);
-        ytop = max(ytop, p.y_min * 15);
-        ybot = min(ybot, p.y_max * 15);
-        if (ybot <= ytop) { ytop = ybot = 0; }
-        f.ytop = ytop; f.ybot = ybot;
-    }
+    edge_span_clamped(e, p, f.ytop, f.ybot);
     f.dir = e.dir; f.fq = 0; f.invW = 0.0; f.fr = 0.0;
     if (p.kind != SWFR_PATH_TOR || e.y2 <= e.y1) { f.ytop = f.ybot = 0; return f; }
     const int64_t DX = (int64_t)e.x2 - e.x1, D = 30ll * ((int64_t)e.y2 - e.y1);
diff --git a/swf_renderer_amd/csrc/renderer.cpp b/swf_renderer_amd/csrc/renderer.cpp
--- a/swf_renderer_amd/csrc/renderer.cpp
+++ b/swf_renderer_amd/csrc/renderer.cpp
@@ -26,7 +26,7 @@
 void launch2_bin(hipStream_t, const Frame2*, uint32_t, uint32_t, uint32_t, uint32_t, uint32_t, bool, uint32_t);
 void launch2_rows(hipStream_t, const Frame2*, uint32_t, uint32_t, uint32_t, bool, bool);
 bool rows_wide_instance(uint32_t, bool);
-void launch2_rows_ahead(hipStream_t, const Frame2*, const Frame2*, uint32_t, uint32_t, uint32_t, uint32_t, uint32_t, uint32_t);
+void launch2_rows_ahead(hipStream_t, const Frame2*, const Frame2*, uint32_t, uint32_t, uint32_t, uint32_t, uint32_t, uint32_t, StageRec* const*, StageRec* const*);
 void launch2_rows_slow(hipStream_t, const Frame2*, uint32_t, uint32_t, uint32_t, uint32_t, bool);
 void launch2_tiles(hipStream_t, const Frame2*, uint32_t, uint32_t, uint32_t, int, uint32_t*);
 void launch2_linear_pieces(hipStream_t, const Frame2*, uint32_t, uint32_t);
@@ -177,6 +177,7 @@
         Frame2 proto{};
         Frame2* frames_dev = nullptr;
         Frame2* frames_ahead = nullptr;
+        StageRec** stage_dev = nullptr;
         uint32_t slow_passes = SLOW_PASSES;
         bool slow_verified = false;
         int slow_state = 0;
@@ -235,6 +236,7 @@
     int bin_threads = 0;
     uint32_t last_bin_threads = 0;
     int bin_ahead = 1;
+    int stage_ahead = 0;
     uint32_t last_ahead_launches = 0;
     int tiles_shaders = 0;
     bool rows_wide = false;
@@ -1150,7 +1152,7 @@
     const FrameDims dims = sc.dims = FrameDims::of_layout(L, a.n_edges, a.n_paths);
     sc.bounds = plan_bounds(L, a.n_edges, a.n_paths);
     SceneArena& A = sc.arena;
-    A.begin(scene_arena_bytes(L, a) + SceneArena::padded(8 * sizeof(Frame2)) + 4096);
+    A.begin(scene_arena_bytes(L, a) + SceneArena::padded(8 * sizeof(Frame2)) + SceneArena::padded(8 * sizeof(StageRec*)) + 4096);
     Frame2 proto;
     std::memset(&proto, 0, sizeof proto);
     push_scene(A, L, a, proto);
@@ -1161,15 +1163,17 @@
     const size_t cls_bytes = cls_region_bytes(dims, tiles_x);
     const int n_sets = std::max(1, std::min(r->in_flight, 4));
     const bool ahead = all_sets && r->bin_ahead && !r->mono && r->cfg.band_count <= 1;
+    const bool staged = ahead && r->stage_ahead;
     Frame2 fr[8];
     std::memset(fr, 0, sizeof fr);
+    StageRec* stage[8] = {nullptr, nullptr, nullptr, nullptr, nullptr, nullptr, nullptr, nullptr};
     for (int k = 0; k < 4; ++k) {
         if (all_sets ? k >= n_sets : k != si) continue;
         auto& x = r->fs[k];
         Frame2& f = fr[k];
         f = proto;
         if (!x.stream) HIP_CHECK(hipStreamCreateWithFlags(&x.stream, hipStreamNonBlocking));
-        x.work.reserve(frame_work_bytes(dims) + (ahead ? frame_ahead_bytes(dims) : 0)); x.cls.reserve(ahead ? pad256(cls_bytes) + cls_bytes : cls_bytes);
+        x.work.reserve(frame_work_bytes(dims) + (ahead ? frame_ahead_bytes(dims) : 0) + (staged ? 2 * stage_rec_bytes(dims) : 0)); x.cls.reserve(ahead ? pad256(cls_bytes) + cls_bytes : cls_bytes);
         uint8_t *w = x.work.ptr, *c = x.cls.ptr;
         place_frame(f, dims, tiles_x, w, c);
         const uint32_t* cost_before = x.strip_cost.ptr;
@@ -1193,10 +1197,12 @@
             if (x.strip_cost_ahead.ptr != cost1_before) HIP_CHECK(hipMemsetAsync(x.strip_cost_ahead.ptr, 0, x.strip_cost_ahead.cap * sizeof(uint32_t), up_stream));
             f1.strip_cost = x.strip_cost_ahead.ptr;
             f1.counters = r->d_counters.ptr + size_t(4 + k) * COUNTER_WORDS;
+            if (staged) { w = carve_stage_recs(stage[k], dims, w); w = carve_stage_recs(stage[4 + k], dims, w); }
         }
     }
     sc.frames_dev = static_cast<Frame2*>(A.push(fr, sizeof fr));
     sc.frames_ahead = ahead ? sc.frames_dev + 4 : nullptr;
+    sc.stage_dev = staged ? static_cast<StageRec**>(A.push(stage, sizeof stage)) : nullptr;
     A.flush(up_stream, si == 0);
     if (all_sets) {
         for (int k = 0; k < n_sets; ++k)
@@ -1444,7 +1450,9 @@
                 }
                 if (gi + groups < launches) {
                     const uint32_t next_cnt = std::min(rb, frames - (f + groups * rb));
-                    launch2_rows_ahead(st, cur, next, cnt, next_cnt, plan.max_edges, plan.max_paths, plan.max_bands, plan.max_chunks);
+                    StageRec* const* st_cur = sc.stage_dev ? sc.stage_dev + (parity ? 4 : 0) + g * rb : nullptr;
+                    StageRec* const* st_next = sc.stage_dev ? sc.stage_dev + (parity ? 0 : 4) + g * rb : nullptr;
+                    launch2_rows_ahead(st, cur, next, cnt, next_cnt, plan.max_edges, plan.max_paths, plan.max_bands, plan.max_chunks, gi >= groups ? st_cur : nullptr, st_next);
                     ++r->last_ahead_launches;
                 } else launch2_rows(st, cur, cnt, plan.max_chunks, plan.max_path_edges, false, false);
                 launch2_tiles(st, cur, cnt, plan.max_strips, plan.tiles_grid, plan.shader_level, nullptr);
@@ -1910,6 +1918,7 @@
 #endif
     if (const char* rb = std::getenv("SWFR_RESIDENT_BATCH")) r->resident_batch = std::atoi(rb);
     if (const char* ba = std::getenv("SWFR_BIN_AHEAD")) r->bin_ahead = std::atoi(ba) != 0;
+    if (const char* sa = std::getenv("SWFR_STAGE_AHEAD")) r->stage_ahead = std::atoi(sa) != 0;
     if (const char* cm = std::getenv("SWFR_CXFORM_CACHE_MB")) r->cx_budget = size_t(std::max(0, std::atoi(cm))) << 20;
     if (r->cfg.device == SWFR_DEVICE_HOST_ONLY) {
         *out = r.release();
diff --git a/swf_renderer_amd/csrc/rows3.hip b/swf_renderer_amd/csrc/rows3.hip
--- a/swf_renderer_amd/csrc/rows3.hip
+++ b/swf_renderer_amd/csrc/rows3.hip
@@ -3,6 +3,9 @@
 #define R3MARK(n) asm volatile("; R3MARK " #n)
 #else
 #define R3MARK(n) do { } while (0)
+#endif
+#ifdef SWFR_EMU
+[[noreturn]] static inline void r3_emu_fail(const char* what) { std::fprintf(stderr, "stage record disagrees with the row pass: %s\n", what); std::abort(); }
 #endif
 template <int STAGE> struct R3Mask { typedef uint32_t type; };
 template <> struct R3Mask<64> { typedef uint64_t type; };
@@ -76,8 +79,8 @@
     while (n < MAX_CELLS_PER_EDGE_ROW) put_cell(dst + n++, xminp, 0, 0, xminp, xmaxp);
 }
 
-template <int STAGE, int NS>
-__device__ __forceinline__ void rows3_chunk_body(FramePtr FR, uint32_t block) {
+template <int STAGE, int NS, bool STAGED = false>
+__device__ __forceinline__ void rows3_chunk_body(FramePtr FR, uint32_t block, const StageRec* __restrict__ recs = nullptr) {
     typedef typename R3Mask<STAGE>::type amask_t;
     __shared__ __attribute__((aligned(16))) FastEdge staged[STAGE];
     __shared__ __attribute__((aligned(16))) uint32_t sub_cells[4][NS * 15];
@@ -85,14 +88,49 @@
     __shared__ uint8_t slot_role[NS][64];
     __shared__ uint8_t slot_edge[NS][64];
     __shared__ uint32_t mid_bits[2];
+#ifdef SWFR_EMU
+    __shared__ uint32_t emu_idx[STAGE];
+#endif
     TRACE_DECL;
     TRACE_NOWAIT(0);
+    R3MARK(13);
     const int lane = threadIdx.x;
     const ChunkInfo ck = FR->chunks[block];
     const uint32_t lo = ck.path;
     const FastEdge* __restrict__ FE = fast_edges_of(FR->edges, FR->n_edges) + ck.first_edge;
-    const FastEdge ek_first = FE[min((uint32_t)lane, ck.n_edges ? ck.n_edges - 1u : 0u)];
-    const DevPath P = FR->paths[lo];
+    uint32_t rec_n = STAGE_REC_NONE, rec_inc = 0, rec_flags = 0, rec_pixel = 0, rec_idx = 0;
+    uint64_t rec_mid = 0, rec_mask = 0;
+    int32_t rec_rect[4] = {0, 0, 0, 0};
+    uint32_t rec_boff[4][2] = {{0u, 0u}, {0u, 0u}, {0u, 0u}, {0u, 0u}};
+    if constexpr (STAGED) {
+        static_assert(STAGE == (int)STAGE_REC_EDGES, "a stage record lists what the staging area holds");
+        if (recs != nullptr) {
+            SWFR_GLOBAL_PTR(const StageRec) rec = (SWFR_GLOBAL_PTR(const StageRec))(recs + block);
+            rec_n = rec->n_list; rec_inc = rec->inc_before; rec_mid = ((uint64_t)rec->mid_hi << 32) | (uint64_t)rec->mid_lo;
+            rec_rect[0] = rec->x_min; rec_rect[1] = rec->x_max; rec_rect[2] = rec->y_min; rec_rect[3] = rec->y_max;
+            rec_flags = rec->flags; rec_pixel = rec->pixel;
+#pragma unroll
+            for (int t = 0; t < 4; ++t) { rec_boff[t][0] = rec->band_off[t][0]; rec_boff[t][1] = rec->band_off[t][1]; }
+            if (lane < (int)STAGE_REC_EDGES) { rec_idx = rec->idx[lane]; rec_mask = rec->mask[lane]; }
+        }
+    }
+    const bool rec_in = STAGED && rec_n != STAGE_REC_NONE;
+#ifdef SWFR_EMU
+    const bool derive = true;
+#else
+    const bool derive = !rec_in;
+#endif
+    const FastEdge ek_first = FE[min(derive ? (uint32_t)lane : 0u, ck.n_edges ? ck.n_edges - 1u : 0u)];
+    DevPath P = {};
+    if (derive) P = FR->paths[lo];
+#ifdef SWFR_EMU
+    const DevPath P_derived = P;
+#endif
+    if (rec_in) {
+        P.first_edge = ck.first_edge; P.n_edges = ck.n_edges; P.kind = (rec_flags & STAGE_REC_TOR) ? (uint32_t)SWFR_PATH_TOR : ~0u;
+        P.fill_rule = rec_flags & STAGE_REC_FILL_RULE; P.style = 0; P.lerp = 0;
+        P.x_min = rec_rect[0]; P.x_max = rec_rect[1]; P.y_min = rec_rect[2]; P.y_max = rec_rect[3];
+    }
     const int r = (int)ck.first_row + lane;
     const int chunk_rows = (int)ck.rows;
 
@@ -103,9 +141,19 @@
     uint32_t cls_b0 = 0, cls_b1 = 0;
     if (ck.slot0 != ~0u && lane < chunk_rows) {
         cls_bs = FR->band_slots[ck.slot0 + (uint32_t)g16];
-        const uint32_t bclamp = min((uint32_t)band, FR->n_bands - 1u);
-        cls_b0 = FR->band_off[bclamp];
-        cls_b1 = FR->band_off[bclamp + 1u];
+        if (derive) {
+            const uint32_t bclamp = min((uint32_t)band, FR->n_bands - 1u);
+            cls_b0 = FR->band_off[bclamp];
+            cls_b1 = FR->band_off[bclamp + 1u];
+        }
+        if (rec_in) {
+            const uint32_t s0 = g16 == 0 ? rec_boff[0][0] : g16 == 1 ? rec_boff[1][0] : g16 == 2 ? rec_boff[2][0] : rec_boff[3][0];
+            const uint32_t s1 = g16 == 0 ? rec_boff[0][1] : g16 == 1 ? rec_boff[1][1] : g16 == 2 ? rec_boff[2][1] : rec_boff[3][1];
+#ifdef SWFR_EMU
+            if (s0 != cls_b0 || s1 != cls_b1) r3_emu_fail("band_off pair");
+#endif
+            cls_b0 = s0; cls_b1 = s1;
+        }
     }
     const bool band_ok = ck.slot0 != ~0u && lane < chunk_rows && band >= band_lo && band <= band_hi && P.kind == SWFR_PATH_TOR;
     const uint32_t ri = band_ok ? cls_bs.slot * TILE_H + (uint32_t)(r & (TILE_H - 1)) : ~0u;
@@ -122,9 +170,14 @@
 #define R3_FIELD(name) ((decltype(FR->name))p_##name)
     const int fast_limit = min((int)FR->fast_limit, NS);
     const int lo_s = (int)ck.first_row * 15, hi_s = lo_s + chunk_rows * 15;
-    if (lane < 2) mid_bits[lane] = 0u;
     uint32_t n_list = 0;
     bool use_lds = true;
+    bool forced_over = false;
+    uint32_t rb_lo = 0, rb_hi = 0;
+    uint32_t chunk_cell_base = 0;
+    uint64_t mid_mask = 0;
+    if (derive) {
+    if (lane < 2) mid_bits[lane] = 0u;
     int inc_before = 0;
     for (uint32_t eb = 0; eb < ck.n_edges; eb += 64) {
         const uint32_t k = eb + (uint32_t)lane;
@@ -135,11 +188,13 @@
         const unsigned long long hb = __ballot(hit);
         const uint32_t at = n_list + (uint32_t)__popcll(hb & ((1ull << lane) - 1ull));
         if (hit && at < (uint32_t)STAGE) staged[at] = ek;
+#ifdef SWFR_EMU
+        if (hit && at < (uint32_t)STAGE) emu_idx[at] = k;
+#endif
         n_list += (uint32_t)__popcll(hb);
         if (n_list > (uint32_t)STAGE) use_lds = false;
     }
-    const uint32_t chunk_cell_base = (ck.rec_base + (uint32_t)__builtin_amdgcn_readlane(wave_scan_incl(inc_before), 63)) * (uint32_t)MAX_CELLS_PER_EDGE_ROW;
-    bool forced_over = false;
+    chunk_cell_base = (ck.rec_base + (uint32_t)__builtin_amdgcn_readlane(wave_scan_incl(inc_before), 63)) * (uint32_t)MAX_CELLS_PER_EDGE_ROW;
     if (!use_lds) {
         int cnt = 0;
         for (uint32_t k = 0; k < P.n_edges; ++k) {
@@ -171,7 +226,6 @@
     lds_barrier();
     SWFR_PIN_SGPR(p_cells); SWFR_PIN_SGPR(p_rows);
     R3MARK(2);
-    uint32_t rb_lo = 0, rb_hi = 0;
     if (use_lds && (uint32_t)lane < n_list) {
         const int yt = staged[lane].ytop, yb = staged[lane].ybot;
         const int ra = yt / 15 - (int)ck.first_row, rz = (yb + 14) / 15 - (int)ck.first_row;
@@ -186,6 +240,33 @@
         if ((uint32_t)(mb >> 32)) atomicOr(&mid_bits[1], (uint32_t)(mb >> 32));
     }
     lds_barrier();
+    mid_mask = ((uint64_t)(uint32_t)__builtin_amdgcn_readfirstlane((int)mid_bits[1]) << 32) | (uint64_t)(uint32_t)__builtin_amdgcn_readfirstlane((int)mid_bits[0]);
+    }
+    if (rec_in) {
+        R3MARK(12);
+        const FastEdge ek_listed = FE[min(rec_idx, ck.n_edges ? ck.n_edges - 1u : 0u)];
+#ifdef SWFR_EMU
+        {
+            const bool listed = (uint32_t)lane < rec_n;
+            if (!use_lds || n_list != rec_n) r3_emu_fail("staged list length");
+            if (listed && (emu_idx[lane] != rec_idx || std::memcmp(&staged[lane], &ek_listed, sizeof ek_listed) != 0)) r3_emu_fail("staged list entry or order");
+            if (listed && (rb_lo != (uint32_t)rec_mask || rb_hi != (uint32_t)(rec_mask >> 32))) r3_emu_fail("row mask");
+            if (mid_mask != rec_mid) r3_emu_fail("mid mask");
+            if (chunk_cell_base != (ck.rec_base + rec_inc) * (uint32_t)MAX_CELLS_PER_EDGE_ROW) r3_emu_fail("inc_before");
+            if (P_derived.kind != P.kind || (P_derived.fill_rule != 0u) != (P.fill_rule != 0u) || P_derived.x_min != P.x_min || P_derived.x_max != P.x_max ||
+                P_derived.y_min != P.y_min || P_derived.y_max != P.y_max || P_derived.n_edges != P.n_edges || P_derived.first_edge != P.first_edge) r3_emu_fail("path rectangle, kind or fill rule");
+            const swfr_style& st = style_at(FR, P_derived.style);
+            if (st.pixel != rec_pixel || (st.kind == SWFR_STYLE_SOLID && P_derived.lerp && (st.pixel >> 24) == 0xffu) != ((rec_flags & STAGE_REC_OPAQUE) != 0u)) r3_emu_fail("style pixel or opaque flag");
+            lds_barrier();
+        }
+#endif
+        n_list = rec_n; use_lds = true; forced_over = false;
+        rb_lo = 0; rb_hi = 0;
+        if ((uint32_t)lane < rec_n) { staged[lane] = ek_listed; rb_lo = (uint32_t)rec_mask; rb_hi = (uint32_t)(rec_mask >> 32); }
+        chunk_cell_base = (ck.rec_base + rec_inc) * (uint32_t)MAX_CELLS_PER_EDGE_ROW;
+        mid_mask = ((uint64_t)(uint32_t)__builtin_amdgcn_readfirstlane((int)(uint32_t)(rec_mid >> 32)) << 32) | (uint64_t)(uint32_t)__builtin_amdgcn_readfirstlane((int)(uint32_t)rec_mid);
+        lds_barrier();
+    }
     TRACE(2);
     R3MARK(3);
     amask_t amask = 0;
@@ -194,7 +275,6 @@
             const uint64_t m = ((uint64_t)(uint32_t)__builtin_amdgcn_readlane((int)rb_hi, k) << 32) | (uint64_t)(uint32_t)__builtin_amdgcn_readlane((int)rb_lo, k);
             amask = (amask_t)(amask << 1) | (amask_t)lane_bit(m, lane);
         }
-    const uint64_t mid_mask = ((uint64_t)(uint32_t)__builtin_amdgcn_readfirstlane((int)mid_bits[1]) << 32) | (uint64_t)(uint32_t)__builtin_amdgcn_readfirstlane((int)mid_bits[0]);
     const bool mid_row = lane_bit(mid_mask, lane) != 0u;
     if (!live) amask = 0;
     int n = r3_count(amask);
@@ -537,8 +617,12 @@
             n_b = cls_b1 - cls_b0;
             out = FR->cls + (size_t)STRIPS_PER_TILE * FR->tiles_x * cls_b0 + (cls_bs.slot - cls_b0);
         }
-        const swfr_style& st = style_at(FR, P.style);
-        const uint32_t opq = (st.kind == SWFR_STYLE_SOLID && P.lerp && (st.pixel >> 24) == 0xffu) ? CLS_OPAQUE : 0u;
+        uint32_t st_pixel, opq;
+        if (rec_in) { st_pixel = rec_pixel; opq = (rec_flags & STAGE_REC_OPAQUE) ? CLS_OPAQUE : 0u; }
+        else {
+            const swfr_style& st = style_at(FR, P.style);
+            st_pixel = st.pixel; opq = (st.kind == SWFR_STYLE_SOLID && P.lerp && (st.pixel >> 24) == 0xffu) ? CLS_OPAQUE : 0u;
+        }
         const bool in_frame = r < height && band_ok, in_rows = in_frame && in_path;
         uint32_t local_trow = 0;
         const bool own_band = band_ok && owns_band(FR, band, local_trow);
@@ -585,7 +669,7 @@
                     out[(uint32_t)(tc * STRIPS_PER_TILE + strip_in_tile) * n_b] = (uint8_t)f;
                     if (own_band) {
                         const uint32_t strip_id = (local_trow * (uint32_t)FR->tiles_x + (uint32_t)tc) * STRIPS_PER_TILE + (uint32_t)strip_in_tile;
-                        strip_top_note(FR, strip_id, pos1, f, st.pixel);
+                        strip_top_note(FR, strip_id, pos1, f, st_pixel);
                         if (cost_order && (f & CLS_PARTIAL)) {
                             const uint32_t wgt = (uint32_t)__popcll((pb >> (lane & ~7)) & 0xffull);
                             if (wgt) atomicAdd(&FR->strip_cost[strip_id], wgt);
@@ -598,4 +682,5 @@
 #undef R3_FIELD
     TRACE(7);
     TRACE_OUT(1, block);
+    R3MARK(14);
 }
```

Result: slower. 402,100 (-1.5%).
